# feiyue126/find_circ2

Hardware: AMD Instinct MI355X
Metric: anchor-pairs/sec (backsplice calls) at 100 bp reads, 1/2/4/8 MI355X (higher is better)
Workload: dtype u32

## Files before the change

find_circ2_amd/_native.py:

```python
from __future__ import annotations

import ctypes
import os
import subprocess

from ._lazy import LazyModule
from ._libpath import LIB_PATH, _HERE

np = LazyModule("numpy", globals(), "np")

FC2_OK = 0
CALLER_MAX_QUEUED = 64
FC2_E_PARAM = -1
FC2_E_HIP = -2
FC2_E_FORMAT = -3
FC2_E_RANGE = -4
FC2_E_IO = -5
FC2_E_KEY = -6
FC2_E_OS = -7

MAX_READ_LEN = 32767

PAIR_BACKSPLICE = 0x01
PAIR_PRIMARY_REV = 0x02
PAIR_READ_N = 0x04
PAIR_BYTEPATH = 0x08
PAIR_SKIP = 0x10
PAIR_WIN_N = 0x20
PAIR_READ_N1 = 0x40

RES_MINUS = 0x0001
RES_GTAG_SHIFT = 1
RES_GTAG_MASK = 0x1FFE
RES_ERR_KEY = 0x2000
RES_ERR_WIN = 0x4000
RES_DONE = 0x8000

_DTYPE_NAMES = ("PAIR_DTYPE", "RESULT_DTYPE", "ESCAPE_DTYPE", "LONG_PAIR_DTYPE", "LONG_RESULT_DTYPE")


def _dtypes():
    PAIR_DTYPE = np.dtype([("a_pos", "<i4"), ("b_aend", "<i4"), ("chrom", "<u4"), ("read_len", "<u2"),
                           ("flags", "u1"), ("npos", "u1")])
    RESULT_DTYPE = np.dtype([("best_x", "<i2"), ("dist", "u1"), ("ov", "u1"), ("n_ties", "<u2"), ("info", "<u2")])
    assert PAIR_DTYPE.itemsize == 16 and RESULT_DTYPE.itemsize == 8
    ESCAPE_DTYPE = np.dtype([("index", "<u8"), ("result", RESULT_DTYPE)])
    LONG_PAIR_DTYPE = np.dtype([("read_off", "<u8"), ("read_len", "<u4"), ("chrom", "<u4"), ("a_pos", "<i4"),
                                ("b_aend", "<i4"), ("flags", "u1"), ("_pad", "u1", (7,))])
    LONG_RESULT_DTYPE = np.dtype([("best_x", "<i4"), ("n_ties", "<u4"), ("dist", "u1"), ("ov", "u1"), ("info", "<u2"),
                                  ("_pad", "<u4")])
    assert LONG_PAIR_DTYPE.itemsize == 32 and LONG_RESULT_DTYPE.itemsize == 16
    g = globals()
    for k in _DTYPE_NAMES:
        g[k] = locals()[k]


def __getattr__(name):
    if name in _DTYPE_NAMES:
        _dtypes()
        return globals()[name]
    raise AttributeError("module %r has no attribute %r" % (__name__, name))
R32_ESCAPE = 0x80000000
R16_ESCAPE = 0x007F


class Fc2Error(RuntimeError):
    def __init__(self, code: int, msg: str):
        super().__init__("libfc2 error %d: %s" % (code, msg))
        self.code = code


class Params(ctypes.Structure):
    _fields_ = [("asize", ctypes.c_int32), ("margin", ctypes.c_int32), ("maxdist", ctypes.c_int32),
                ("noncanonical", ctypes.c_uint8), ("strandpref", ctypes.c_uint8),
                ("allhits", ctypes.c_uint8), ("_pad", ctypes.c_uint8)]


class GenomeView(ctypes.Structure):
    _fields_ = [("units", ctypes.c_void_p), ("nplane", ctypes.c_void_p), ("ncoarse", ctypes.c_void_p),
                ("chrom_start", ctypes.c_void_p), ("chrom_size", ctypes.c_void_p),
                ("n_units", ctypes.c_uint64), ("n_chrom", ctypes.c_uint32), ("dummy", ctypes.c_uint32),
                ("units_twin", ctypes.c_void_p), ("nsuper", ctypes.c_void_p), ("nsuper_shift", ctypes.c_uint32),
                ("nsuper_words", ctypes.c_uint32), ("wt", ctypes.c_void_p), ("wt_bytes", ctypes.c_uint64),
                ("wt_twin_off", ctypes.c_uint64)]


class BatchView(ctypes.Structure):
    _fields_ = [("pairs", ctypes.c_void_p), ("read_words", ctypes.c_void_p), ("read_nwords", ctypes.c_void_p),
                ("n", ctypes.c_uint64), ("stride", ctypes.c_uint64), ("rw", ctypes.c_uint32),
                ("nw", ctypes.c_uint32), ("max_l", ctypes.c_int32), ("layout", ctypes.c_uint32),
                ("win_words", ctypes.c_void_p), ("win_nwords", ctypes.c_void_p), ("ww", ctypes.c_uint32),
                ("wnw", ctypes.c_uint32)]


BATCH_LOCUS_ORDERED = 0x1
BATCH_FORM_STAGED = 0x02
BATCH_FORM_PLAIN = 0x04
BATCH_FORM_UNITS = 0x08
BATCH_FORM_TWOLANE = 0x10
BATCH_FORM_TRI = 0x20
BATCH_FORM_FIVE = 0x40
BATCH_FORM_WAVE = 0x80


class CompactOut(ctypes.Structure):
    _fields_ = [("width", ctypes.c_int32), ("esc_cap", ctypes.c_uint32), ("words", ctypes.c_void_p),
                ("esc", ctypes.c_void_p), ("esc_count", ctypes.c_void_p), ("count_out", ctypes.c_void_p)]


class ReorderInfo(ctypes.Structure):
    _fields_ = [("n", ctypes.c_uint64), ("workspace_bytes", ctypes.c_uint64), ("shift", ctypes.c_uint32),
                ("n_buckets", ctypes.c_uint32), ("bucket_bits", ctypes.c_uint32), ("n_chunks", ctypes.c_uint32),
                ("n_groups", ctypes.c_uint32), ("chunk", ctypes.c_uint32)]


class BytesView(ctypes.Structure):
    _fields_ = [("index", ctypes.c_void_p), ("pairs", ctypes.c_void_p), ("arena", ctypes.c_void_p),
                ("off", ctypes.c_void_p), ("m", ctypes.c_uint64)]


class SynthCfg(ctypes.Structure):
    _fields_ = [("seed", ctypes.c_uint64), ("len_min", ctypes.c_int32), ("len_max", ctypes.c_int32),
                ("p_planted", ctypes.c_float), ("p_minus_site", ctypes.c_float),
                ("p_backsplice", ctypes.c_float), ("mut_rate", ctypes.c_float), ("n_rate", ctypes.c_float),
                ("p_clip", ctypes.c_float), ("span_min", ctypes.c_int32), ("span_max", ctypes.c_int32),
                ("locus_ordered", ctypes.c_int32), ("p_three_seg", ctypes.c_float), ("first", ctypes.c_uint64)]


EXPORTED = [
    "fc2_abi_version", "fc2_last_error", "fc2_device_count", "fc2_host_register", "fc2_host_unregister", "fc2_set_tuning", "fc2_get_tuning", "fc2_max_fast_l",
    "fc2_batch_geometry",
    "fc2_bp_scan_launch", "fc2_bp_scan_bytes_launch", "fc2_probe_pattern_launch",
    "fc2_result_compact_launch", "fc2_result_expand", "fc2_bp_scan_compact_launch", "fc2_host_device_pointer",
    "fc2_fasta_open", "fc2_fasta_close", "fc2_fasta_n_chrom", "fc2_fasta_chrom", "fc2_fasta_find",
    "fc2_fasta_get_upper", "fc2_fasta_layout", "fc2_fasta_pack", "fc2_fasta_prepack",
    "fc2_pack_pairs", "fc2_bytepath_size", "fc2_bytepath_fill", "fc2_window_geometry", "fc2_pack_windows",
    "fc2_gather_windows_launch", "fc2_long_geometry", "fc2_long_fill", "fc2_bp_scan_long_launch",
    "fc2_synth_genome_launch", "fc2_coarse_launch", "fc2_twin_launch", "fc2_wtab_geometry", "fc2_wtab_launch",
    "fc2_nsuper_geometry", "fc2_nsuper_launch", "fc2_synth_pairs_launch",
    "fc2_reorder_plan", "fc2_reorder_launch",
    "fc2_ingest_open", "fc2_ingest_close", "fc2_ingest_n_refs", "fc2_ingest_ref_name", "fc2_ingest_header",
    "fc2_ingest_next", "fc2_ingest_counts_get", "fc2_ingest_set_bam_out", "fc2_ingest_close_bam_out",
    "fc2_ingest_format", "fc2_sam_to_bam", "fc2_bgzf_inflate_launch",
    "fc2_ingest_set_gpu_inflate", "fc2_ingest_set_gpu_inflate_from", "fc2_ingest_inflate_counts",
    "fc2_bam_walk_launch", "fc2_bam_walk_host", "fc2_ingest_set_gpu_walk", "fc2_ingest_walk_counts",
    "fc2_bam_digest_launch", "fc2_bam_digest_host", "fc2_ingest_set_gpu_digest", "fc2_ingest_digest_counts",
    "fc2_caller_open", "fc2_caller_set_genome", "fc2_caller_inflate_counts", "fc2_caller_ingest", "fc2_caller_close", "fc2_caller_next",
    "fc2_caller_submit", "fc2_caller_submit_compact", "fc2_caller_submit_long", "fc2_caller_queued", "fc2_caller_take", "fc2_caller_rows", "fc2_caller_write_rows", "fc2_caller_counter", "fc2_caller_stats",
    "fc2_caller_set_reads_gz", "fc2_caller_close_reads", "fc2_caller_set_reads_gz_device", "fc2_caller_reads_gz_counts",
    "fc2_deflate_launch", "fc2_deflate_scratch_bytes", "fc2_gpu_gzip", "fc2_gpu_gzip_bound", "fc2_caller_set_reads_gz_device_tuning",
    "fc2_ctx_create", "fc2_ctx_create_sibling", "fc2_ctx_destroy", "fc2_ctx_genome_load", "fc2_ctx_genome_view", "fc2_ctx_scan_async",
    "fc2_ctx_sync", "fc2_ctx_scan_long", "fc2_ctx_stream", "fc2_ctx_last_error",
]


BAM_WALK_CAP = 1824
BAM_WALK_NO_EXIT = 0xFFFFFFFF
BAM_DIGEST_MAX_BLOCKS = 1024


class BamDigest(ctypes.Structure):
    _fields_ = [("state", ctypes.c_uint8), ("as_type", ctypes.c_uint8), ("xs_type", ctypes.c_uint8),
                ("has_qual", ctypes.c_uint8), ("block_size", ctypes.c_uint32), ("astart", ctypes.c_int32),
                ("qlen", ctypes.c_int32), ("as_bits", ctypes.c_uint32), ("xs_bits", ctypes.c_uint32),
                ("aend", ctypes.c_int64)]


class IngestParams(ctypes.Structure):
    _fields_ = [("asize", ctypes.c_int32), ("nolinear", ctypes.c_uint8), ("noop", ctypes.c_uint8),
                ("_pad", ctypes.c_uint8 * 2)]


class IngestCounts(ctypes.Structure):
    _fields_ = [("n_reads", ctypes.c_uint64), ("total_mates", ctypes.c_uint64), ("unmapped_reads", ctypes.c_uint64),
                ("unspliced_mates", ctypes.c_uint64), ("seg_too_short_skip", ctypes.c_uint64),
                ("records", ctypes.c_uint64), ("handed_back", ctypes.c_uint64)]

class CallerOpts(ctypes.Structure):
    _fields_ = [("name", ctypes.c_char_p), ("known_circ", ctypes.c_char_p), ("known_lin", ctypes.c_char_p),
                ("min_uniq_qual", ctypes.c_int32), ("asize", ctypes.c_int32), ("margin", ctypes.c_int32),
                ("maxdist", ctypes.c_int32), ("short_threshold", ctypes.c_int32), ("huge_threshold", ctypes.c_int32),
                ("noncanonical", ctypes.c_uint8), ("allhits", ctypes.c_uint8), ("stranded", ctypes.c_uint8),
                ("strandpref", ctypes.c_uint8), ("halfunique", ctypes.c_uint8), ("report_nobridges", ctypes.c_uint8),
                ("test", ctypes.c_uint8), ("nolinear", ctypes.c_uint8), ("multi_events", ctypes.c_uint8),
                ("noop", ctypes.c_uint8), ("write_reads", ctypes.c_uint8), ("write_multi", ctypes.c_uint8),
                ("_pad", ctypes.c_uint32), ("chunksize", ctypes.c_uint64)]


class CallerBatch(ctypes.Structure):
    _fields_ = [("n", ctypes.c_uint64), ("reads", ctypes.c_void_p), ("read_off", ctypes.c_void_p),
                ("pairs", ctypes.c_void_p), ("n_long", ctypes.c_uint64), ("long_pairs", ctypes.c_void_p)]


_lib = None


def build(force: bool = False) -> str:
    srcdir = os.path.join(_HERE, "csrc")
    srcs = [os.path.join(srcdir, f) for f in ("fc2_kernels.hip", "fc2_scan32.hip", "fc2_reorder.hip", "fc2_inflate.hip",
                                              "fc2_deflate.hip", "fc2_deflate_gpu.hip", "fc2_deflate_gpu.h", "fc2_devcrc.h",
                                              "fc2_gzpieces.h", "fc2_scan32.h",
                                              "fc2_host.cpp", "fc2_ingest.cpp", "fc2_ingest_impl.h", "fc2_caller.cpp",
                                              "fc2_bamout.cpp", "fc2_bamout.h", "fc2_ctx.cpp", "fc2_hostmem.h",
                                              "fc2_common.h", "Makefile")]
    srcs += [os.path.join(os.path.dirname(_HERE), "include", h)
             for h in ("fc2_bp.h", "fc2_ingest.h", "fc2_caller.h", "fc2_ctx.h")]
    newest = max(os.path.getmtime(s) for s in srcs)
    if force or not os.path.exists(LIB_PATH) or os.path.getmtime(LIB_PATH) < newest:
        subprocess.check_call(["make", "-s", "-C", srcdir])
    return LIB_PATH


def lib() -> ctypes.CDLL:
    global _lib
    if _lib is not None:
        return _lib
    if not os.path.exists(LIB_PATH):
        raise ImportError("libfc2.so is not built (%s); run __graft_entry__.build() -- there is no CPU fallback"
                          % LIB_PATH)
    L = ctypes.CDLL(LIB_PATH)
    vp, u64, u32, i32, i64 = ctypes.c_void_p, ctypes.c_uint64, ctypes.c_uint32, ctypes.c_int32, ctypes.c_int64
    P = ctypes.POINTER
    sig = {
        "fc2_abi_version": (ctypes.c_int, []),
        "fc2_last_error": (ctypes.c_char_p, []),
        "fc2_device_count": (ctypes.c_int, [P(ctypes.c_int)]),
        "fc2_max_fast_l": (ctypes.c_int, []),
        "fc2_host_register": (ctypes.c_int, [vp, u64]),
        "fc2_host_unregister": (ctypes.c_int, [vp]),
        "fc2_set_tuning": (ctypes.c_int, [ctypes.c_int, ctypes.c_int]),
        "fc2_get_tuning": (ctypes.c_int, [ctypes.c_int, ctypes.POINTER(ctypes.c_int)]),
        "fc2_batch_geometry": (ctypes.c_int, [P(Params), i32, P(u32), P(u32), P(u32)]),
        "fc2_bp_scan_launch": (ctypes.c_int, [P(Params), P(GenomeView), P(BatchView), vp, vp, u32, vp]),
        "fc2_bp_scan_bytes_launch": (ctypes.c_int, [P(Params), P(BytesView), vp, vp, u32, u64, vp]),
        "fc2_probe_pattern_launch": (ctypes.c_int, [P(Params), P(GenomeView), P(BatchView), vp, vp]),
        "fc2_result_compact_launch": (ctypes.c_int, [P(Params), vp, u64, ctypes.c_int, vp, vp, u32, vp, vp]),
        "fc2_result_expand": (ctypes.c_int, [P(Params), vp, ctypes.c_int, u64, vp, u64, vp, ctypes.c_int]),
        "fc2_bp_scan_compact_launch": (ctypes.c_int, [P(Params), P(GenomeView), P(BatchView), P(CompactOut), vp]),
        "fc2_host_device_pointer": (ctypes.c_int, [vp, P(vp)]),
        "fc2_fasta_open": (ctypes.c_int, [ctypes.c_char_p, ctypes.c_int, P(vp)]),
        "fc2_fasta_close": (None, [vp]),
        "fc2_fasta_n_chrom": (ctypes.c_int, [vp]),
        "fc2_fasta_chrom": (ctypes.c_int, [vp, ctypes.c_int, P(ctypes.c_char_p), P(i64), P(i64), P(i64),
                                           P(i64), P(ctypes.c_int)]),
        "fc2_fasta_find": (ctypes.c_int, [vp, ctypes.c_char_p]),
        "fc2_fasta_get_upper": (ctypes.c_int, [vp, ctypes.c_int, i64, i64, vp, i64, P(i64)]),
        "fc2_fasta_layout": (ctypes.c_int, [vp, P(u64), P(u64), vp]),
        "fc2_fasta_pack": (ctypes.c_int, [vp, vp, vp, vp, P(u64), ctypes.c_int]),
        "fc2_fasta_prepack": (ctypes.c_int, [vp, ctypes.c_int]),
        "fc2_pack_pairs": (ctypes.c_int, [P(Params), vp, u64, vp, vp, vp, vp, u32, vp, u32, u64, P(u64),
                                          ctypes.c_int]),
        "fc2_bytepath_size": (ctypes.c_int, [P(Params), u64, vp, P(u64), P(u64)]),
        "fc2_window_geometry": (ctypes.c_int, [P(Params), ctypes.c_int, P(u32), P(u32), P(u32)]),
        "fc2_pack_windows": (ctypes.c_int, [P(Params), vp, u64, vp, vp, vp, u32, u64, ctypes.c_int]),
        "fc2_gather_windows_launch": (ctypes.c_int, [P(Params), P(GenomeView), P(BatchView), vp, vp, vp, u32, vp]),
        "fc2_bytepath_fill": (ctypes.c_int, [P(Params), vp, u64, vp, vp, vp, vp, vp, vp, vp]),
        "fc2_long_geometry": (ctypes.c_int, [P(Params), u64, vp, P(ctypes.c_uint64), vp]),
        "fc2_long_fill": (ctypes.c_int, [P(Params), vp, u64, vp, vp, vp, vp]),
        "fc2_bp_scan_long_launch": (ctypes.c_int, [P(Params), u64, vp, vp, vp, vp, vp, vp, vp]),
        "fc2_synth_genome_launch": (ctypes.c_int, [u64, vp, vp, vp, u64, vp, vp, u32, vp]),
        "fc2_coarse_launch": (ctypes.c_int, [vp, vp, u64, vp]),
        "fc2_twin_launch": (ctypes.c_int, [vp, u64, vp, vp]),
        "fc2_wtab_geometry": (ctypes.c_int, [u64, P(u64), P(u64)]),
        "fc2_wtab_launch": (ctypes.c_int, [vp, u64, vp, vp]),
        "fc2_nsuper_geometry": (ctypes.c_int, [u64, P(u32), P(u32)]),
        "fc2_nsuper_launch": (ctypes.c_int, [vp, u64, vp, vp]),
        "fc2_synth_pairs_launch": (ctypes.c_int, [P(Params), P(SynthCfg), P(GenomeView), vp, u64, vp, vp, u32,
                                                  vp, u32, u64, vp, vp]),
        "fc2_reorder_plan": (ctypes.c_int, [P(GenomeView), u64, P(ReorderInfo)]),
        "fc2_reorder_launch": (ctypes.c_int, [P(ReorderInfo), P(GenomeView), P(BatchView), vp, vp, vp, vp, vp, vp]),
        "fc2_ingest_open": (ctypes.c_int, [ctypes.c_char_p, ctypes.c_int, P(vp)]),
        "fc2_ingest_close": (None, [vp]),
        "fc2_ingest_n_refs": (ctypes.c_int, [vp]),
        "fc2_ingest_ref_name": (ctypes.c_char_p, [vp, ctypes.c_int]),
        "fc2_ingest_header": (ctypes.c_char_p, [vp]),
        "fc2_ingest_next": (ctypes.c_int, [vp, P(IngestParams), u64, P(IngestCounts), P(ctypes.c_void_p), P(u64),
                                           P(u64), P(ctypes.c_int)]),
        "fc2_ingest_counts_get": (ctypes.c_int, [vp, P(IngestCounts)]),
        "fc2_ingest_set_bam_out": (ctypes.c_int, [vp, ctypes.c_char_p]),
        "fc2_ingest_close_bam_out": (ctypes.c_int, [vp]),
        "fc2_ingest_format": (ctypes.c_int, [vp, P(ctypes.c_int)]),
        "fc2_sam_to_bam": (ctypes.c_int, [ctypes.c_char_p, ctypes.c_char_p]),
        "fc2_caller_open": (ctypes.c_int, [ctypes.c_char_p, ctypes.c_int, P(CallerOpts), P(vp)]),
        "fc2_caller_set_genome": (ctypes.c_int, [vp, vp, i32, vp, P(u64), P(u64)]),
        "fc2_caller_ingest": (vp, [vp]),
        "fc2_caller_close": (None, [vp]),
        "fc2_caller_next": (ctypes.c_int, [vp, P(CallerBatch), P(ctypes.c_int)]),
        "fc2_caller_submit": (ctypes.c_int, [vp, vp, vp, u32, u64]),
        "fc2_caller_submit_compact": (ctypes.c_int, [vp, vp, ctypes.c_int, u64, vp, u64, vp, u32, u64]),
        "fc2_caller_submit_long": (ctypes.c_int, [vp, vp, u64, vp, u64]),
        "fc2_caller_queued": (ctypes.c_int, [vp]),
        "fc2_caller_take": (ctypes.c_int, [vp, ctypes.c_int, P(ctypes.c_void_p), P(u64)]),
        "fc2_caller_set_reads_gz": (ctypes.c_int, [vp, ctypes.c_char_p, ctypes.c_int, ctypes.c_int, u64]),
        "fc2_caller_close_reads": (ctypes.c_int, [vp]),
        "fc2_caller_set_reads_gz_device": (ctypes.c_int, [vp, ctypes.c_int]),
        "fc2_caller_reads_gz_counts": (ctypes.c_int, [vp, P(u64), P(u64)]),
        "fc2_deflate_launch": (ctypes.c_int, [vp, u64, u32, vp, u32, vp, vp, vp, vp]),
        "fc2_deflate_scratch_bytes": (u64, [u64, u32]),
        "fc2_gpu_gzip": (ctypes.c_int, [ctypes.c_int, vp, u64, u32, vp, u64, P(u64)]),
        "fc2_gpu_gzip_bound": (u64, [u64, u32]),
        "fc2_caller_set_reads_gz_device_tuning": (ctypes.c_int, [vp, u32, ctypes.c_double]),
        "fc2_caller_rows": (ctypes.c_int, [vp, ctypes.c_int, P(ctypes.c_void_p), P(u64)]),
        "fc2_caller_write_rows": (ctypes.c_int, [vp, ctypes.c_int, ctypes.c_int, P(u64)]),
        "fc2_caller_counter": (ctypes.c_int, [vp, ctypes.c_int, P(ctypes.c_char_p), P(ctypes.c_double)]),
        "fc2_caller_stats": (ctypes.c_int, [vp, P(u64), P(u64)]),
        "fc2_bgzf_inflate_launch": (ctypes.c_int, [vp, vp, vp, vp, vp, vp, vp, u32, vp]),
        "fc2_ingest_set_gpu_inflate": (ctypes.c_int, [vp, ctypes.c_int, ctypes.c_int]),
        "fc2_ingest_set_gpu_inflate_from": (ctypes.c_int, [vp, ctypes.c_int, u64]),
        "fc2_ingest_inflate_counts": (ctypes.c_int, [vp, P(u64), P(u64)]),
        "fc2_bam_walk_launch": (ctypes.c_int, [vp, vp, vp, vp, vp, vp, u32, vp]),
        "fc2_bam_walk_host": (ctypes.c_int, [vp, u32, vp, P(u32), P(u32)]),
        "fc2_ingest_set_gpu_walk": (ctypes.c_int, [vp, ctypes.c_int]),
        "fc2_ingest_walk_counts": (ctypes.c_int, [vp, P(u64), P(u64)]),
        "fc2_bam_digest_launch": (ctypes.c_int, [vp, u32, vp, vp, vp, vp, vp, vp, vp, u32, vp]),
        "fc2_bam_digest_host": (ctypes.c_int, [vp, u32, u32, P(BamDigest)]),
        "fc2_ingest_set_gpu_digest": (ctypes.c_int, [vp, ctypes.c_int]),
        "fc2_ingest_digest_counts": (ctypes.c_int, [vp, P(u64), P(u64)]),
        "fc2_caller_inflate_counts": (ctypes.c_int, [vp, P(u64), P(u64)]),
        "fc2_ctx_create": (ctypes.c_int, [ctypes.c_int, P(vp)]),
        "fc2_ctx_create_sibling": (ctypes.c_int, [vp, P(vp)]),
        "fc2_ctx_destroy": (None, [vp]),
        "fc2_ctx_genome_load": (ctypes.c_int, [vp, vp, ctypes.c_int]),
        "fc2_ctx_genome_view": (ctypes.c_int, [vp, P(GenomeView)]),
        "fc2_ctx_scan_async": (ctypes.c_int, [vp, P(Params), u64, vp, vp, vp, vp, vp, u32, ctypes.c_int]),
        "fc2_ctx_sync": (ctypes.c_int, [vp]),
        "fc2_ctx_scan_long": (ctypes.c_int, [vp, P(Params), u64, vp, vp, vp, vp]),
        "fc2_ctx_stream": (vp, [vp]),
        "fc2_ctx_last_error": (ctypes.c_char_p, [vp]),
    }
    for name, (res, args) in sig.items():
        if os.environ.get("FC2_LIB_VARIANT") and not hasattr(L, name):
            continue
        fn = getattr(L, name)
        fn.restype = res
        fn.argtypes = args
    if L.fc2_abi_version() != 1:
        raise ImportError("libfc2.so ABI mismatch")
    _lib = L
    return L


def get_tuning(key: int) -> int:
    v = ctypes.c_int(0)
    check(lib().fc2_get_tuning(key, ctypes.byref(v)))
    return v.value


def check(rc: int) -> None:
    if rc != FC2_OK:
        msg = lib().fc2_last_error()
        raise Fc2Error(rc, msg.decode("utf-8", "replace") if msg else "")


def ptr(a) -> int:
    if a is None:
        return None
    if isinstance(a, np.ndarray):
        return a.ctypes.data
    return a.data_ptr()
```

find_circ2_amd/csrc/fc2_ctx.cpp:

```cpp
#include <hip/hip_runtime.h>
#include <stdio.h>
#include <stdlib.h>
#include <string.h>
#include <sys/mman.h>

#include <algorithm>
#include <chrono>
#include <memory>
#include <string>
#include <vector>

#include "../../include/fc2_bp.h"
#include "../../include/fc2_ctx.h"
#include "fc2_common.h"
#include "fc2_hostmem.h"

namespace {

int hip_fail(hipError_t e, const char *what) {
    return fc2::fail(FC2_E_HIP, std::string(what) + ": " + hipGetErrorString(e));
}

struct DevBuf {
    void *p = nullptr;
    size_t cap = 0;
    int reserve(size_t bytes, const char *what, bool slack = true) {
        if (bytes <= cap && p) return FC2_OK;
        if (p) (void)hipFree(p);
        p = nullptr;
        cap = 0;
        const size_t want = std::max<size_t>(slack ? bytes + bytes / 4 : bytes, 256);
        const hipError_t e = hipMalloc(&p, want);
        if (e != hipSuccess) { p = nullptr; return hip_fail(e, what); }
        cap = want;
        return FC2_OK;
    }
    void release() {
        if (p) (void)hipFree(p);
        p = nullptr;
        cap = 0;
    }
    template <class T> T *as() const { return static_cast<T *>(p); }
};

struct HostBuf {
    void *p = nullptr;
    size_t cap = 0;
    int reserve(size_t bytes, const char *what) {
        if (bytes <= cap && p) return FC2_OK;
        if (p) (void)hipHostFree(p);
        p = nullptr;
        cap = 0;
        const size_t want = std::max<size_t>(bytes + bytes / 4, 256);
        const hipError_t e = hipHostMalloc(&p, want, hipHostMallocDefault);
        if (e != hipSuccess) { p = nullptr; return hip_fail(e, what); }
        cap = want;
        return FC2_OK;
    }
    void release() {
        if (p) (void)hipHostFree(p);
        p = nullptr;
        cap = 0;
    }
    template <class T> T *as() const { return static_cast<T *>(p); }
};

}

struct fc2_ctx {
    int device = 0;
    hipStream_t stream = nullptr;
    std::string err;
    bool have_genome = false;
    bool borrowed = false;
    const fc2_fasta *fa = nullptr;
    fc2_genome_view gv{};
    DevBuf units, nplane, ncoarse, cstart, csize, twin, nsuper, wt;
    fc2::MappedWords h_units, h_nplane;
    HostBuf h_pairs, h_words, h_nwords, h_res, h_tm, h_bidx, h_bpairs, h_boff, h_arena;
    DevBuf d_pairs, d_words, d_nwords, d_res, d_tm, d_bidx, d_bpairs, d_boff, d_arena;
    bool pending = false;
    uint64_t n = 0;
    uint32_t tw = 0;
    bool allhits = false;
    fc2_result *out_res = nullptr;
    uint64_t *out_tm = nullptr;

    void free_genome() {
        if (!borrowed)
            for (DevBuf *b : {&units, &nplane, &ncoarse, &cstart, &csize, &twin, &nsuper, &wt}) b->release();
        h_units.release();
        h_nplane.release();
        borrowed = false;
        gv = fc2_genome_view{};
        have_genome = false;
        fa = nullptr;
    }
};

namespace {

int keep(fc2_ctx *c, int rc) {
    if (rc != FC2_OK && c) {
        const char *m = fc2_last_error();
        c->err = m ? m : "";
    }
    return rc;
}

int use_device(fc2_ctx *c) {
    const hipError_t e = hipSetDevice(c->device);
    return e == hipSuccess ? FC2_OK : hip_fail(e, "hipSetDevice");
}

int h2d(DevBuf &d, const void *src, size_t bytes, hipStream_t s) {
    if (!bytes) return FC2_OK;
    const hipError_t e = hipMemcpyAsync(d.p, src, bytes, hipMemcpyHostToDevice, s);
    return e == hipSuccess ? FC2_OK : hip_fail(e, "hipMemcpyAsync H2D");
}

}

extern "C" int fc2_ctx_create(int device, fc2_ctx **out) {
    if (!out) return fc2::fail(FC2_E_PARAM, "fc2_ctx_create: null argument");
    *out = nullptr;
    if (device < 0) return fc2::fail(FC2_E_PARAM, "fc2_ctx_create: negative device");
    int count = 0;
    hipError_t e = hipGetDeviceCount(&count);
    if (e != hipSuccess) return hip_fail(e, "fc2_ctx_create: hipGetDeviceCount");
    if (device >= count)
        return fc2::fail(FC2_E_HIP, "fc2_ctx_create: device " + std::to_string(device) + " of " +
                                        std::to_string(count));
    fc2_ctx *c = new fc2_ctx();
    c->device = device;
    int rc = use_device(c);
    if (rc == FC2_OK) {
        e = hipStreamCreateWithFlags(&c->stream, hipStreamNonBlocking);
        if (e != hipSuccess) rc = hip_fail(e, "hipStreamCreateWithFlags");
    }
    if (rc != FC2_OK) {
        delete c;
        return rc;
    }
    *out = c;
    return FC2_OK;
}

extern "C" int fc2_ctx_create_sibling(const fc2_ctx *src, fc2_ctx **out) {
    if (!src || !out) return fc2::fail(FC2_E_PARAM, "fc2_ctx_create_sibling: null argument");
    *out = nullptr;
    if (!src->have_genome) return fc2::fail(FC2_E_PARAM, "fc2_ctx_create_sibling: the source context has no genome");
    fc2_ctx *c = nullptr;
    if (int rc = fc2_ctx_create(src->device, &c)) return rc;
    c->gv = src->gv;
    c->fa = src->fa;
    c->have_genome = true;
    c->borrowed = true;
    *out = c;
    return FC2_OK;
}

extern "C" void fc2_ctx_destroy(fc2_ctx *c) {
    if (!c) return;
    if (hipSetDevice(c->device) == hipSuccess && c->stream) (void)hipStreamSynchronize(c->stream);
    c->free_genome();
    for (HostBuf *b : {&c->h_pairs, &c->h_words, &c->h_nwords, &c->h_res, &c->h_tm, &c->h_bidx, &c->h_bpairs,
                       &c->h_boff, &c->h_arena})
        b->release();
    for (DevBuf *b : {&c->d_pairs, &c->d_words, &c->d_nwords, &c->d_res, &c->d_tm, &c->d_bidx, &c->d_bpairs,
                      &c->d_boff, &c->d_arena})
        b->release();
    if (c->stream) (void)hipStreamDestroy(c->stream);
    delete c;
}

extern "C" int fc2_ctx_genome_load(fc2_ctx *c, const fc2_fasta *fa, int n_threads) {
    if (!c) return fc2::fail(FC2_E_PARAM, "fc2_ctx_genome_load: null context");
    c->err.clear();
    if (c->pending) return keep(c, fc2::fail(FC2_E_PARAM, "fc2_ctx_genome_load: a batch is queued (fc2_ctx_sync)"));
    int rc = use_device(c);
    if (rc) return keep(c, rc);
    if (hipStreamSynchronize(c->stream) != hipSuccess) return keep(c, fc2::fail(FC2_E_HIP, "stream sync"));
    c->free_genome();
    if (!fa) {
        c->gv.dummy = 1;
        c->gv.n_chrom = 0xFFFFFFFFu;
        c->have_genome = true;
        return FC2_OK;
    }
    static const bool timing = getenv("FC2_CALLER_TIMING") != nullptr;
    const auto t0 = std::chrono::steady_clock::now();
    auto ms = [&] { return std::chrono::duration<double, std::milli>(std::chrono::steady_clock::now() - t0).count(); };
    const int nch = fc2_fasta_n_chrom(fa);
    std::vector<int64_t> sizes((size_t)std::max(nch, 1), 0);
    for (int i = 0; i < nch; ++i)
        if ((rc = fc2_fasta_chrom(fa, i, nullptr, &sizes[(size_t)i], nullptr, nullptr, nullptr, nullptr))) return keep(c, rc);
    uint64_t nu = 0, ncw = 0;
    std::vector<uint64_t> cs((size_t)std::max(nch, 1), 0);
    if ((rc = fc2_fasta_layout(fa, &nu, &ncw, cs.data()))) return keep(c, rc);
    fc2::MappedWords &units = c->h_units, &nplane = c->h_nplane;
    std::vector<uint32_t> ncoarse;
    uint64_t n_exotic = 0;
    const bool prepacked = fc2::take_prepacked(fa, nu, units, nplane, ncoarse);
    if (!prepacked) {
        units = fc2::MappedWords(2 * nu);
        nplane = fc2::MappedWords(nu);
    }
    if (!units.ok() || !nplane.ok()) return keep(c, fc2::fail(FC2_E_OS, "fc2_ctx_genome_load: cannot map host memory for the 2-bit genome"));
    const double t_alloc = ms();
    if (!prepacked) {
        ncoarse.assign((size_t)std::max<uint64_t>(ncw, 1), 0);
        if ((rc = fc2_fasta_pack(fa, units.data(), nplane.data(), ncoarse.data(), &n_exotic, n_threads))) return keep(c, rc);
    }
    const double t_pack = ms();
    const hipStream_t s = c->stream;
    if ((rc = c->units.reserve(units.size() * 8, "genome units", false)) || (rc = c->nplane.reserve(nplane.size() * 8, "genome N plane", false)) ||
        (rc = c->ncoarse.reserve(ncoarse.size() * 4, "genome coarse N map", false)) || (rc = c->cstart.reserve(cs.size() * 8, "chromosome starts", false)) ||
        (rc = c->csize.reserve(sizes.size() * 8, "chromosome sizes", false)) || (rc = c->twin.reserve(2 * (nu + 8) * 8, "genome twin", false)))
        return keep(c, rc);
    if ((rc = h2d(c->units, units.data(), units.size() * 8, s)) || (rc = h2d(c->nplane, nplane.data(), nplane.size() * 8, s)) ||
        (rc = h2d(c->ncoarse, ncoarse.data(), ncoarse.size() * 4, s)) || (rc = h2d(c->cstart, cs.data(), cs.size() * 8, s)) ||
        (rc = h2d(c->csize, sizes.data(), sizes.size() * 8, s)))
        return keep(c, rc);
    if ((rc = fc2_twin_launch(c->units.as<uint64_t>(), nu, c->twin.as<uint64_t>(), s))) return keep(c, rc);
    uint32_t ns_shift = 0, ns_words = 0;
    if ((rc = fc2_nsuper_geometry(nu, &ns_shift, &ns_words))) return keep(c, rc);
    const size_t ns_alloc = ((size_t)ns_words + 3) / 4 * 4;
    if ((rc = c->nsuper.reserve(ns_alloc * 4, "N super map", false))) return keep(c, rc);
    if (hipMemsetAsync(c->nsuper.p, 0, ns_alloc * 4, s) != hipSuccess) return keep(c, fc2::fail(FC2_E_HIP, "memset"));
    if ((rc = fc2_nsuper_launch(c->ncoarse.as<uint32_t>(), nu, c->nsuper.as<uint32_t>(), s))) return keep(c, rc);
    uint64_t wt_bytes = 0, wt_twin_off = 0;
    const bool words = fc2_wtab_geometry(nu, &wt_bytes, &wt_twin_off) == FC2_OK;
    if (words) {
        if ((rc = c->wt.reserve(wt_bytes, "word-pair table", false))) return keep(c, rc);
        if ((rc = fc2_wtab_launch(c->units.as<uint64_t>(), nu, c->wt.as<uint32_t>(), s))) return keep(c, rc);
    }
    const hipError_t e = hipStreamSynchronize(s);
    if (e != hipSuccess) return keep(c, hip_fail(e, "genome upload"));
    if (timing)
        fprintf(stderr, "genome load: host vectors %.1f ms, 2-bit pack %.1f ms%s, device alloc + upload + tables %.1f ms "
                        "(%llu units)\n", t_alloc, t_pack - t_alloc, prepacked ? " (prepacked)" : "", ms() - t_pack,
                (unsigned long long)nu);
    fc2_genome_view &g = c->gv;
    g.units = c->units.as<const uint64_t>();
    g.nplane = c->nplane.as<const uint64_t>();
    g.ncoarse = c->ncoarse.as<const uint32_t>();
    g.chrom_start = c->cstart.as<const uint64_t>();
    g.chrom_size = c->csize.as<const int64_t>();
    g.n_units = nu;
    g.n_chrom = (uint32_t)nch;
    g.dummy = 0;
    g.units_twin = c->twin.as<const uint64_t>();
    g.nsuper = c->nsuper.as<const uint32_t>();
    g.nsuper_shift = ns_shift;
    g.nsuper_words = ns_words;
    g.wt = words ? c->wt.as<const uint32_t>() : nullptr;
    g.wt_bytes = words ? wt_bytes : 0;
    g.wt_twin_off = words ? wt_twin_off : 0;
    c->fa = fa;
    c->have_genome = true;
    return FC2_OK;
}

extern "C" int fc2_ctx_genome_view(const fc2_ctx *c, fc2_genome_view *out) {
    if (!c || !out) return fc2::fail(FC2_E_PARAM, "fc2_ctx_genome_view: null argument");
    if (!c->have_genome) return fc2::fail(FC2_E_PARAM, "fc2_ctx_genome_view: no genome loaded");
    *out = c->gv;
    return FC2_OK;
}

extern "C" int fc2_ctx_scan_async(fc2_ctx *c, const fc2_params *p, uint64_t n, const uint8_t *reads,
                                  const uint64_t *read_off, const fc2_pair *pairs, fc2_result *results,
                                  uint64_t *tiemask, uint32_t tw, int n_threads) {
    if (!c) return fc2::fail(FC2_E_PARAM, "fc2_ctx_scan_async: null context");
    c->err.clear();
    int rc = fc2::validate_params(p);
    if (rc) return keep(c, rc);
    if (c->pending) return keep(c, fc2::fail(FC2_E_PARAM, "fc2_ctx_scan_async: the previous batch was not synced"));
    if (!c->have_genome)
        return keep(c, fc2::fail(FC2_E_PARAM, "fc2_ctx_scan_async: no genome (fc2_ctx_genome_load; NULL = dummy genome)"));
    if (n && (!reads || !read_off || !pairs || !results))
        return keep(c, fc2::fail(FC2_E_PARAM, "fc2_ctx_scan_async: null argument"));
    if (p->allhits && n && !tiemask) return keep(c, fc2::fail(FC2_E_PARAM, "fc2_ctx_scan_async: --all-hits needs a tie mask"));
    if ((rc = use_device(c))) return keep(c, rc);
    c->n = n;
    c->allhits = p->allhits != 0;
    c->tw = tw;
    c->out_res = results;
    c->out_tm = tiemask;
    if (n == 0) {
        c->pending = true;
        return FC2_OK;
    }
    int max_len = 0;
    for (uint64_t i = 0; i < n; ++i) max_len = std::max<int>(max_len, pairs[i].read_len);
    uint32_t rw = 0, nw = 0, tw_need = 0;
    if ((rc = fc2_batch_geometry(p, max_len, &rw, &nw, &tw_need))) return keep(c, rc);
    if (c->allhits && tw < tw_need)
        return keep(c, fc2::fail(FC2_E_PARAM, "fc2_ctx_scan_async: tie mask of " + std::to_string(tw) + " words per pair, " +
                                                  std::to_string(tw_need) + " needed"));
    const size_t tmw = c->allhits ? (size_t)tw * n : 0;
    if ((rc = c->h_pairs.reserve(n * sizeof(fc2_pair), "pair staging")) || (rc = c->h_words.reserve((size_t)rw * n * 8, "read-row staging")) ||
        (rc = c->h_nwords.reserve((size_t)nw * n * 8, "N-row staging")) || (rc = c->h_res.reserve(n * 8, "result staging")) ||
        (tmw && (rc = c->h_tm.reserve(tmw * 8, "tie-mask staging"))) || (rc = c->d_pairs.reserve(n * sizeof(fc2_pair), "pairs")) ||
        (rc = c->d_words.reserve((size_t)rw * n * 8, "read rows")) || (rc = c->d_nwords.reserve((size_t)nw * n * 8, "N rows")) ||
        (rc = c->d_res.reserve(n * 8, "results")) || (tmw && (rc = c->d_tm.reserve(tmw * 8, "tie mask"))))
        return keep(c, rc);
    memcpy(c->h_pairs.p, pairs, n * sizeof(fc2_pair));
    memset(c->h_words.p, 0, (size_t)rw * n * 8);
    memset(c->h_nwords.p, 0, (size_t)nw * n * 8);
    fc2_pair *hp = c->h_pairs.as<fc2_pair>();
    uint64_t n_bytepath = 0;
    if ((rc = fc2_pack_pairs(p, c->fa, n, reads, read_off, hp, c->h_words.as<uint64_t>(), rw, c->h_nwords.as<uint64_t>(), nw,
                             n, &n_bytepath, n_threads)))
        return keep(c, rc);
    const int e = fc2::eff_anchor(p);
    int max_l = 0;
    for (uint64_t i = 0; i < n; ++i)
        if (!(hp[i].flags & (FC2_PAIR_BYTEPATH | FC2_PAIR_SKIP))) max_l = std::max(max_l, (int)hp[i].read_len - 2 * e);
    const hipStream_t s = c->stream;
    auto abandon = [&](int code) {
        const std::string msg = fc2_last_error();
        (void)hipStreamSynchronize(s);
        return keep(c, fc2::fail(code, msg));
    };
    if ((rc = h2d(c->d_pairs, hp, n * sizeof(fc2_pair), s)) || (rc = h2d(c->d_words, c->h_words.p, (size_t)rw * n * 8, s)) ||
        (rc = h2d(c->d_nwords, c->h_nwords.p, (size_t)nw * n * 8, s)))
        return abandon(rc);
    if (tmw && hipMemsetAsync(c->d_tm.p, 0, tmw * 8, s) != hipSuccess) return abandon(fc2::fail(FC2_E_HIP, "tie-mask memset"));
    fc2_batch_view bv{};
    bv.pairs = c->d_pairs.as<const fc2_pair>();
    bv.read_words = c->d_words.as<const uint64_t>();
    bv.read_nwords = c->d_nwords.as<const uint64_t>();
    bv.n = n;
    bv.stride = n;
    bv.rw = rw;
    bv.nw = nw;
    bv.max_l = max_l;
    bv.layout = 0;
    uint64_t *dtm = tmw ? c->d_tm.as<uint64_t>() : nullptr;
    if ((rc = fc2_bp_scan_launch(p, &c->gv, &bv, c->d_res.as<fc2_result>(), dtm, tw, s))) return abandon(rc);
    if (n_bytepath) {
        uint64_t m = 0, arena = 0;
        if ((rc = fc2_bytepath_size(p, n, hp, &m, &arena))) return abandon(rc);
        if ((rc = c->h_bidx.reserve(m * 8, "byte-path index")) || (rc = c->h_bpairs.reserve(m * sizeof(fc2_pair), "byte-path pairs")) ||
            (rc = c->h_boff.reserve(m * 8, "byte-path offsets")) || (rc = c->h_arena.reserve(std::max<uint64_t>(arena, 16), "byte-path arena")) ||
            (rc = c->d_bidx.reserve(m * 8, "byte-path index")) || (rc = c->d_bpairs.reserve(m * sizeof(fc2_pair), "byte-path pairs")) ||
            (rc = c->d_boff.reserve(m * 8, "byte-path offsets")) || (rc = c->d_arena.reserve(std::max<uint64_t>(arena, 16), "byte-path arena")))
            return abandon(rc);
        if ((rc = fc2_bytepath_fill(p, c->fa, n, reads, read_off, hp, c->h_bidx.as<uint64_t>(), c->h_bpairs.as<fc2_pair>(),
                                    c->h_boff.as<uint64_t>(), c->h_arena.as<uint8_t>())))
            return abandon(rc);
        if ((rc = h2d(c->d_bidx, c->h_bidx.p, m * 8, s)) || (rc = h2d(c->d_bpairs, c->h_bpairs.p, m * sizeof(fc2_pair), s)) ||
            (rc = h2d(c->d_boff, c->h_boff.p, m * 8, s)) || (rc = h2d(c->d_arena, c->h_arena.p, arena, s)))
            return abandon(rc);
        fc2_bytes_view v{c->d_bidx.as<const uint64_t>(), c->d_bpairs.as<const fc2_pair>(), c->d_arena.as<const uint8_t>(),
                         c->d_boff.as<const uint64_t>(), m};
        if ((rc = fc2_bp_scan_bytes_launch(p, &v, c->d_res.as<fc2_result>(), dtm, tw, n, s))) return abandon(rc);
    }
    hipError_t he = hipMemcpyAsync(c->h_res.p, c->d_res.p, n * 8, hipMemcpyDeviceToHost, s);
    if (he == hipSuccess && tmw) he = hipMemcpyAsync(c->h_tm.p, c->d_tm.p, tmw * 8, hipMemcpyDeviceToHost, s);
    if (he != hipSuccess) return abandon(hip_fail(he, "hipMemcpyAsync D2H"));
    c->pending = true;
    return FC2_OK;
}

extern "C" int fc2_ctx_sync(fc2_ctx *c) {
    if (!c) return fc2::fail(FC2_E_PARAM, "fc2_ctx_sync: null context");
    c->err.clear();
    if (!c->pending) return FC2_OK;
    c->pending = false;
    int rc = use_device(c);
    if (rc) return keep(c, rc);
    const hipError_t e = hipStreamSynchronize(c->stream);
    if (e != hipSuccess) return keep(c, hip_fail(e, "fc2_ctx_sync"));
    if (c->n) {
        memcpy(c->out_res, c->h_res.p, c->n * 8);
        if (c->allhits) memcpy(c->out_tm, c->h_tm.p, (size_t)c->tw * c->n * 8);
    }
    return FC2_OK;
}

extern "C" int fc2_ctx_scan_long(fc2_ctx *c, const fc2_params *p, uint64_t n, const uint8_t *reads,
                                 const fc2_long_pair *pairs, fc2_long_result *results, uint64_t *ties) {
    if (!c) return fc2::fail(FC2_E_PARAM, "fc2_ctx_scan_long: null context");
    c->err.clear();
    int rc = fc2::validate_params(p);
    if (rc) return keep(c, rc);
    if (c->pending) return keep(c, fc2::fail(FC2_E_PARAM, "fc2_ctx_scan_long: a batch is queued (fc2_ctx_sync)"));
    if (!c->have_genome)
        return keep(c, fc2::fail(FC2_E_PARAM, "fc2_ctx_scan_long: no genome (fc2_ctx_genome_load; NULL = dummy genome)"));
    if (n == 0) return FC2_OK;
    if (!reads || !pairs || !results || (p->allhits && !ties))
        return keep(c, fc2::fail(FC2_E_PARAM, "fc2_ctx_scan_long: null argument"));
    if ((rc = use_device(c))) return keep(c, rc);
    uint64_t arena = 0;
    std::vector<uint64_t> tie_off(n + 1), off(n);
    if ((rc = fc2_long_geometry(p, n, pairs, &arena, tie_off.data()))) return keep(c, rc);
    std::vector<uint8_t> h_arena((size_t)std::max<uint64_t>(arena, 16));
    if ((rc = fc2_long_fill(p, c->fa, n, reads, pairs, off.data(), h_arena.data()))) return keep(c, rc);
    const uint64_t nt = p->allhits ? tie_off[n] : 0;
    DevBuf d_lp, d_off, d_arena, d_toff, d_res, d_ties;
    auto cleanup = [&] { for (DevBuf *b : {&d_lp, &d_off, &d_arena, &d_toff, &d_res, &d_ties}) b->release(); };
    const hipStream_t s = c->stream;
    if ((rc = d_lp.reserve(n * sizeof(fc2_long_pair), "long pairs", false)) || (rc = d_off.reserve(n * 8, "long offsets", false)) ||
        (rc = d_arena.reserve(h_arena.size(), "long arena", false)) || (rc = d_toff.reserve((n + 1) * 8, "long tie offsets", false)) ||
        (rc = d_res.reserve(n * sizeof(fc2_long_result), "long results", false)) ||
        (nt && (rc = d_ties.reserve(nt * 8, "long ties", false)))) {
        cleanup();
        return keep(c, rc);
    }
    if ((rc = h2d(d_lp, pairs, n * sizeof(fc2_long_pair), s)) || (rc = h2d(d_off, off.data(), n * 8, s)) ||
        (rc = h2d(d_arena, h_arena.data(), h_arena.size(), s)) || (rc = h2d(d_toff, tie_off.data(), (n + 1) * 8, s)) ||
        (rc = fc2_bp_scan_long_launch(p, n, d_lp.as<fc2_long_pair>(), d_off.as<uint64_t>(), d_arena.as<uint8_t>(),
                                      d_toff.as<uint64_t>(), d_res.as<fc2_long_result>(), nt ? d_ties.as<uint64_t>() : nullptr, s))) {
        (void)hipStreamSynchronize(s);
        cleanup();
        return keep(c, rc);
    }
    hipError_t he = hipMemcpyAsync(results, d_res.p, n * sizeof(fc2_long_result), hipMemcpyDeviceToHost, s);
    if (he == hipSuccess && nt) he = hipMemcpyAsync(ties, d_ties.p, nt * 8, hipMemcpyDeviceToHost, s);
    const hipError_t se = hipStreamSynchronize(s);
    cleanup();
    if (he != hipSuccess) return keep(c, hip_fail(he, "fc2_ctx_scan_long D2H"));
    if (se != hipSuccess) return keep(c, hip_fail(se, "fc2_ctx_scan_long"));
    return FC2_OK;
}

extern "C" void *fc2_ctx_stream(const fc2_ctx *c) { return c ? (void *)c->stream : nullptr; }

extern "C" const char *fc2_ctx_last_error(const fc2_ctx *c) { return c ? c->err.c_str() : ""; }
```

find_circ2_amd/csrc/fc2_host.cpp:

```cpp
#include <errno.h>
#include <fcntl.h>
#include <stdio.h>
#include <stdlib.h>
#include <string.h>
#include <sys/mman.h>
#include <sys/stat.h>
#include <unistd.h>
#include <immintrin.h>

#include <algorithm>
#include <atomic>
#include <chrono>
#include <functional>
#include <memory>
#include <string>
#include <thread>
#include <unordered_map>
#include <vector>

#include "fc2_common.h"
#include "fc2_compact.h"
#include "fc2_hostmem.h"

namespace fc2 {

static thread_local std::string g_err;

void set_error(const std::string &msg) { g_err = msg; }
int fail(int code, const std::string &msg) {
    g_err = msg;
    return code;
}

int validate_params(const fc2_params *p) {
    if (!p) return fail(FC2_E_PARAM, "null fc2_params");
    if ((int64_t)p->asize - p->margin < -65536)
        return fail(FC2_E_RANGE, "asize - margin < -65536 is not supported (windows of over 128k bases per pair)");
    if (p->margin > 255) return fail(FC2_E_RANGE, "margin > 255 is not supported (ov is stored in 8 bits)");
    return FC2_OK;
}

static int n_workers(int n_threads) {
    if (n_threads > 0) return n_threads;
    unsigned h = std::thread::hardware_concurrency();
    const char *env = getenv("OMP_NUM_THREADS");
    if (env && atoi(env) > 0) h = (unsigned)atoi(env);
    if (h == 0) h = 1;
    if (h > 64) h = 64;
    return (int)h;
}

static void parallel_for(uint64_t n, int threads, const std::function<void(uint64_t, uint64_t)> &body) {
    if (n == 0) return;
    if (threads <= 1 || n < 4096) {
        body(0, n);
        return;
    }
    uint64_t t = (uint64_t)threads;
    if (t > n) t = n;
    std::vector<std::thread> pool;
    pool.reserve(t);
    for (uint64_t k = 0; k < t; ++k) {
        const uint64_t b = n * k / t, e = n * (k + 1) / t;
        pool.emplace_back([&body, b, e] { body(b, e); });
    }
    for (auto &th : pool) th.join();
}

static inline uint8_t upc(uint8_t c) { return (c >= 'a' && c <= 'z') ? (uint8_t)(c - 32) : c; }

static inline int bclass(uint8_t c) {
    switch (upc(c)) {
        case 'A': return 0;
        case 'C': return 1;
        case 'G': return 2;
        case 'T': return 3;
        case 'N': return 4;
        default: return 5;
    }
}

struct PackTable {
    uint8_t t[256];
    PackTable() {
        for (int c = 0; c < 256; ++c) {
            const int cl = bclass((uint8_t)c);
            t[c] = (uint8_t)(cl < 4 ? cl : cl == 4 ? 4 : 4 | 8);
        }
    }
};
static const PackTable kPackTable;
static inline uint32_t pack_code(uint8_t c) { return kPackTable.t[c]; }

struct BaseMasks {
    uint64_t a, c, g, t, n, nl;
};

static inline BaseMasks base_masks_scalar(const uint8_t *s, int len) {
    BaseMasks m{0, 0, 0, 0, 0, 0};
    for (int j = 0; j < len; ++j) {
        const uint64_t bit = 1ull << j;
        if (s[j] == '\n') m.nl |= bit;
        switch (s[j] & 0xDF) {
            case 'A': m.a |= bit; break;
            case 'C': m.c |= bit; break;
            case 'G': m.g |= bit; break;
            case 'T': m.t |= bit; break;
            case 'N': m.n |= bit; break;
            default: break;
        }
    }
    return m;
}

__attribute__((target("avx2"))) static BaseMasks base_masks_avx2(const uint8_t *s) {
    const __m256i up = _mm256_set1_epi8((char)0xDF);
    const __m256i r0 = _mm256_loadu_si256((const __m256i *)s), r1 = _mm256_loadu_si256((const __m256i *)(s + 32));
    const __m256i v0 = _mm256_and_si256(r0, up), v1 = _mm256_and_si256(r1, up);
#define FC2_MASK64(x0, x1, ch)                                                                             \
    ((uint64_t)(uint32_t)_mm256_movemask_epi8(_mm256_cmpeq_epi8(x0, _mm256_set1_epi8(ch))) |                 \
     (uint64_t)(uint32_t)_mm256_movemask_epi8(_mm256_cmpeq_epi8(x1, _mm256_set1_epi8(ch))) << 32)
    const BaseMasks m{FC2_MASK64(v0, v1, 'A'), FC2_MASK64(v0, v1, 'C'), FC2_MASK64(v0, v1, 'G'),
                      FC2_MASK64(v0, v1, 'T'), FC2_MASK64(v0, v1, 'N'), FC2_MASK64(r0, r1, '\n')};
#undef FC2_MASK64
    return m;
}

#if defined(__HIP_DEVICE_COMPILE__)
static const bool kHaveAvx2 = false;
#else
static const bool kHaveAvx2 = (__builtin_cpu_init(), __builtin_cpu_supports("avx2"));
#endif

static inline bool acgt8(uint64_t u) {
    auto zero = [](uint64_t y) { return ~(((y & 0x7F7F7F7F7F7F7F7Full) + 0x7F7F7F7F7F7F7F7Full) | y | 0x7F7F7F7F7F7F7F7Full); };
    const uint64_t m = zero(u ^ 0x4141414141414141ull) | zero(u ^ 0x4343434343434343ull) |
                       zero(u ^ 0x4747474747474747ull) | zero(u ^ 0x5454545454545454ull);
    return m == 0x8080808080808080ull;
}

static inline bool py_isspace(uint8_t c) {
    return c == ' ' || c == '\t' || c == '\n' || c == '\r' || c == '\v' || c == '\f';
}

}

using namespace fc2;

struct fc2_chrom_rec {
    std::string name;
    int64_t ofs = 0, ldata = 0, skip = 0, size = 0;
    std::string skipchar;
    int nfields = 4;
    int regular = -1;
    uint64_t gstart = 0;
};

struct fc2_fasta {
    std::string path;
    int fd = -1;
    const uint8_t *data = nullptr;
    size_t n = 0;
    std::vector<fc2_chrom_rec> chroms;
    std::unordered_map<std::string, int> by_name;
    std::vector<uint64_t> exotic;
    bool packed = false;
    struct Prepacked {
        fc2::MappedWords units, nplane;
        std::vector<uint32_t> ncoarse;
        uint64_t n_units = 0;
    };
    std::unique_ptr<Prepacked> prepacked;
};

static int build_index(fc2_fasta *f) {
    std::unordered_map<std::string, int> &idx = f->by_name;
    std::vector<fc2_chrom_rec> &cs = f->chroms;
    int64_t ofs = 0, chrom_ofs = 0, size = 0;
    std::string chrom = "undef";
    const uint8_t *d = f->data;
    const size_t n = f->n;
    size_t i = 0;
    while (i < n) {
        const uint8_t *nl = (const uint8_t *)memchr(d + i, '\n', n - i);
        const size_t j = nl ? (size_t)(nl - d) + 1 : n;
        const uint8_t *line = d + i;
        const int64_t len = (int64_t)(j - i);
        ofs += len;
        if (line[0] == '>') {
            if (size) {
                auto it = idx.find(chrom);
                if (it == idx.end())
                    return fail(FC2_E_FORMAT, "FASTA header without sequence before '" + chrom +
                                                  "': reference indexed_fasta.index raises KeyError");
                cs[it->second].size = size;
                cs[it->second].nfields += 1;
            }
            int64_t s = 1;
            while (s < len && py_isspace(line[s])) ++s;
            int64_t e = s;
            while (e < len && !py_isspace(line[e])) ++e;
            if (e == s) return fail(FC2_E_FORMAT, "empty FASTA header: reference raises IndexError");
            chrom.assign((const char *)line + s, (size_t)(e - s));
            chrom_ofs = ofs;
        } else {
            int64_t a = 0, b = len;
            while (a < b && py_isspace(line[a])) ++a;
            while (b > a && py_isspace(line[b - 1])) --b;
            const int64_t stripped = b - a;
            if (idx.find(chrom) == idx.end()) {
                size = 0;
                fc2_chrom_rec r;
                r.name = chrom;
                r.ofs = chrom_ofs;
                r.ldata = stripped;
                r.skip = len - stripped;
                r.skipchar.assign((const char *)line + stripped, (size_t)(len - stripped));
                idx[chrom] = (int)cs.size();
                cs.push_back(r);
            }
            size += stripped;
        }
        i = j;
    }
    if (size) {
        auto it = idx.find(chrom);
        if (it != idx.end()) {
            cs[it->second].size = size;
            cs[it->second].nfields += 1;
        }
    }
    for (auto &c : cs)
        if (c.nfields != 5)
            return fail(FC2_E_FORMAT, "chromosome '" + c.name +
                                          "' has an inconsistent index entry (empty or duplicated sequence); "
                                          "the reference's store_index/get_data fail on it");
    return FC2_OK;
}

static std::string py2_repr(const std::string &s) {
    std::string o = "'";
    for (unsigned char c : s) {
        if (c == '\n') o += "\\n";
        else if (c == '\r') o += "\\r";
        else if (c == '\t') o += "\\t";
        else if (c == '\'') o += "\\'";
        else if (c == '\\') o += "\\\\";
        else if (c >= 32 && c < 127) o += (char)c;
        else {
            char buf[8];
            snprintf(buf, sizeof buf, "\\x%02x", c);
            o += buf;
        }
    }
    return o + "'";
}

static bool py2_unescape(const std::string &in, std::string &out) {
    out.clear();
    for (size_t i = 0; i < in.size(); ++i) {
        char c = in[i];
        if (c != '\\') { out += c; continue; }
        if (++i >= in.size()) return false;
        switch (in[i]) {
            case 'n': out += '\n'; break;
            case 'r': out += '\r'; break;
            case 't': out += '\t'; break;
            case '\\': out += '\\'; break;
            case '\'': out += '\''; break;
            case '"': out += '"'; break;
            case 'x': {
                if (i + 2 >= in.size()) return false;
                out += (char)strtol(in.substr(i + 1, 2).c_str(), nullptr, 16);
                i += 2;
                break;
            }
            default: out += '\\'; out += in[i];
        }
    }
    return true;
}

static int load_index_file(fc2_fasta *f, const std::string &ipath) {
    FILE *fp = fopen(ipath.c_str(), "r");
    if (!fp) return fail(FC2_E_IO, "cannot open index: IOError: [Errno " + std::to_string(errno) + "] " +
                                       strerror(errno) + ": '" + ipath + "'");
    char *line = nullptr;
    size_t cap = 0;
    ssize_t len;
    int rc = FC2_OK;
    while ((len = getline(&line, &cap, fp)) > 0) {
        std::string s(line, (size_t)len);
        while (!s.empty() && py_isspace((uint8_t)s.back())) s.pop_back();
        std::vector<std::string> parts;
        size_t st = 0;
        for (;;) {
            size_t t = s.find('\t', st);
            parts.push_back(s.substr(st, t == std::string::npos ? std::string::npos : t - st));
            if (t == std::string::npos) break;
            st = t + 1;
        }
        if (parts.size() != 6 || parts[4].size() < 2) { rc = fail(FC2_E_FORMAT, "malformed .byo_index line: " + s); break; }
        fc2_chrom_rec r;
        r.name = parts[0];
        r.ofs = atoll(parts[1].c_str());
        r.ldata = atoll(parts[2].c_str());
        r.skip = atoll(parts[3].c_str());
        if (!py2_unescape(parts[4].substr(1, parts[4].size() - 2), r.skipchar)) { rc = fail(FC2_E_FORMAT, "bad skipchar in .byo_index"); break; }
        r.size = atoll(parts[5].c_str());
        r.nfields = 5;
        f->by_name[r.name] = (int)f->chroms.size();
        f->chroms.push_back(r);
    }
    free(line);
    fclose(fp);
    std::stable_sort(f->chroms.begin(), f->chroms.end(),
                     [](const fc2_chrom_rec &a, const fc2_chrom_rec &b) { return a.ofs < b.ofs; });
    f->by_name.clear();
    for (size_t i = 0; i < f->chroms.size(); ++i) f->by_name[f->chroms[i].name] = (int)i;
    return rc;
}

static int store_index_file(const fc2_fasta *f, const std::string &ipath) {
    std::vector<const fc2_chrom_rec *> v;
    for (auto &c : f->chroms) v.push_back(&c);
    std::sort(v.begin(), v.end(), [](const fc2_chrom_rec *a, const fc2_chrom_rec *b) { return a->name < b->name; });
    std::string dir = ipath.substr(0, ipath.find_last_of('/') == std::string::npos ? 0 : ipath.find_last_of('/') + 1);
    std::string tmpl = (dir.empty() ? std::string("./") : dir) + "tmpXXXXXX";
    std::vector<char> buf(tmpl.begin(), tmpl.end());
    buf.push_back(0);
    auto oserror = [&](int err, const char *what) {
        return fail(FC2_E_OS, std::string("OSError: [Errno ") + std::to_string(err) + "] " + strerror(err) + ": '" +
                                  what + "' (writing the FASTA index " + ipath + ")");
    };
    int fd = mkstemp(buf.data());
    if (fd < 0) return oserror(errno, tmpl.c_str());
    std::string body;
    for (auto *c : v) {
        char num[128];
        body += c->name;
        snprintf(num, sizeof num, "\t%lld\t%lld\t%lld\t", (long long)c->ofs, (long long)c->ldata, (long long)c->skip);
        body += num;
        body += py2_repr(c->skipchar);
        snprintf(num, sizeof num, "\t%lld\n", (long long)c->size);
        body += num;
    }
    size_t done = 0;
    while (done < body.size()) {
        const ssize_t w = write(fd, body.data() + done, body.size() - done);
        if (w < 0) {
            if (errno == EINTR) continue;
            const int err = errno;
            close(fd);
            unlink(buf.data());
            return oserror(err, buf.data());
        }
        done += (size_t)w;
    }
    if (fsync(fd) != 0) { const int err = errno; close(fd); unlink(buf.data()); return oserror(err, buf.data()); }
    close(fd);
    if (chmod(buf.data(), S_IRUSR | S_IRGRP | S_IROTH) != 0) { const int err = errno; unlink(buf.data()); return oserror(err, buf.data()); }
    if (rename(buf.data(), ipath.c_str()) != 0) { const int err = errno; unlink(buf.data()); return oserror(err, buf.data()); }
    return FC2_OK;
}

static inline int64_t floordiv(int64_t a, int64_t b) {
    int64_t q = a / b;
    if ((a % b != 0) && ((a < 0) != (b < 0))) --q;
    return q;
}
static inline int64_t pyclip(int64_t i, int64_t n) {
    if (i < 0) { i += n; if (i < 0) i = 0; }
    return i > n ? n : i;
}

static int get_upper_impl(const fc2_fasta *f, int ci, int64_t start, int64_t end, std::string &out,
                          size_t limit = SIZE_MAX, int64_t *full_len = nullptr, int tail_char = -1,
                          int64_t *tail_mis = nullptr) {
    out.clear();
    if (tail_mis) *tail_mis = 0;
    if (!f) {
        if (end > start) out.assign(std::min((size_t)(end - start), limit), 'N');
        const int64_t full = end > start ? end - start : 0;
        if (full_len) *full_len = full;
        if (tail_mis && tail_char != 'N' && full > (int64_t)limit) *tail_mis = full - (int64_t)limit;
        return FC2_OK;
    }
    if (ci < 0 || ci >= (int)f->chroms.size()) return fail(FC2_E_KEY, "unknown chromosome index");
    const fc2_chrom_rec &c = f->chroms[ci];
    if (c.ldata == 0) return fail(FC2_E_FORMAT, "chromosome '" + c.name + "' has ldata 0: reference raises ZeroDivisionError");
    int64_t pad_start = 0, pad_end = 0;
    if (start < 0) { pad_start = -start; start = 0; }
    if (end > c.size) { pad_end = end - c.size; end = c.size; }
    const int64_t os = pyclip(floordiv(start, c.ldata) * c.skip + start + c.ofs, (int64_t)f->n);
    const int64_t oe = pyclip(floordiv(end, c.ldata) * c.skip + end + c.ofs, (int64_t)f->n);
    const uint64_t full = (uint64_t)pad_start + (uint64_t)pad_end + (uint64_t)(oe > os ? oe - os : 0);
    if (limit == SIZE_MAX && full > (1ull << 32))
        return fail(FC2_E_RANGE, "window of " + std::to_string(full) + " bytes from chromosome '" + c.name +
                                     "': the reference's get_data raises MemoryError");
    out.reserve(std::min((size_t)full, limit));
    out.append(std::min((size_t)pad_start, limit), 'N');
    const size_t sl = c.skipchar.size();
    for (int64_t p = os; p < oe && out.size() < limit;) {
        if (sl && p + (int64_t)sl <= oe && !memcmp(f->data + p, c.skipchar.data(), sl)) { p += (int64_t)sl; continue; }
        out.push_back((char)upc(f->data[p]));
        ++p;
    }
    out.append(std::min((size_t)pad_end, limit - out.size()), 'N');
    if (full_len || tail_mis) {
        const int64_t lim = limit == SIZE_MAX ? INT64_MAX : (int64_t)limit;
        int64_t k = pad_start, mis = 0;
        const bool n_differs = tail_char != 'N';
        if (n_differs && pad_start > lim) mis += pad_start - lim;
        for (int64_t p = os; p < oe;) {
            if (sl && p + (int64_t)sl <= oe && !memcmp(f->data + p, c.skipchar.data(), sl)) { p += (int64_t)sl; continue; }
            if (k >= lim && (int)upc(f->data[p]) != tail_char) ++mis;
            ++k;
            ++p;
        }
        if (n_differs) mis += std::max<int64_t>(0, k + pad_end - std::max(k, lim));
        if (full_len) *full_len = k + pad_end;
        if (tail_mis) *tail_mis = mis;
    }
    return FC2_OK;
}

extern "C" int fc2_abi_version(void) { return FC2_ABI_VERSION; }
extern "C" const char *fc2_last_error(void) { return g_err.c_str(); }
extern "C" int fc2_max_fast_l(void) { return kMaxFastL; }

extern "C" int fc2_batch_geometry(const fc2_params *p, int32_t max_read_len, uint32_t *rw, uint32_t *nw, uint32_t *tw) {
    int rc = validate_params(p);
    if (rc) return rc;
    int lmax = max_read_len - 2 * eff_anchor(p);
    if (lmax < 0) lmax = 0;
    const int lfast = lmax > kMaxFastL ? kMaxFastL : lmax;
    if (rw) *rw = (uint32_t)std::max(1, (2 * lfast + 63) / 64);
    if (nw) *nw = (uint32_t)std::max(1, (lfast + 63) / 64);
    if (tw) *tw = (uint32_t)(2 * std::max(1, (lmax + 2 + 63) / 64));
    return FC2_OK;
}

extern "C" int fc2_fasta_open(const char *path, int write_index, fc2_fasta **out) {
    if (!path || !out) return fail(FC2_E_PARAM, "fc2_fasta_open: null argument");
    *out = nullptr;
    auto ioerror = [&](int err) {
        return fail(FC2_E_IO, std::string("cannot open FASTA: IOError: [Errno ") + std::to_string(err) + "] " +
                                  strerror(err) + ": '" + path + "'");
    };
    int fd = open(path, O_RDONLY);
    if (fd < 0) return ioerror(errno);
    struct stat st;
    if (fstat(fd, &st) != 0) { const int err = errno; close(fd); return ioerror(err); }
    if (S_ISDIR(st.st_mode)) { close(fd); return ioerror(EISDIR); }
    fc2_fasta *f = new fc2_fasta();
    f->path = path;
    f->fd = fd;
    f->n = (size_t)st.st_size;
    if (f->n) {
        void *m = mmap(nullptr, f->n, PROT_READ, MAP_SHARED, fd, 0);
        if (m == MAP_FAILED) {
            const int err = errno;
            close(fd);
            delete f;
            return fail(FC2_E_OS, std::string("mmap.error: [Errno ") + std::to_string(err) + "] " + strerror(err) +
                                      " (FASTA '" + path + "')");
        }
        f->data = (const uint8_t *)m;
        madvise(m, f->n, MADV_WILLNEED);
    }
    const std::string ipath = std::string(path) + ".byo_index";
    int rc;
    if (access(ipath.c_str(), R_OK) == 0) {
        rc = load_index_file(f, ipath);
    } else {
        rc = build_index(f);
        if (rc == FC2_OK && write_index) rc = store_index_file(f, ipath);
    }
    if (rc != FC2_OK) { fc2_fasta_close(f); return rc; }
    *out = f;
    return FC2_OK;
}

extern "C" void fc2_fasta_close(fc2_fasta *f) {
    if (!f) return;
    if (f->data) munmap((void *)f->data, f->n);
    if (f->fd >= 0) close(f->fd);
    delete f;
}

extern "C" int fc2_fasta_n_chrom(const fc2_fasta *f) { return f ? (int)f->chroms.size() : 0; }

extern "C" int fc2_fasta_chrom(const fc2_fasta *f, int i, const char **name, int64_t *size, int64_t *ofs, int64_t *ldata,
                               int64_t *skip, int *regular) {
    if (!f || i < 0 || i >= (int)f->chroms.size()) return fail(FC2_E_PARAM, "fc2_fasta_chrom: bad index");
    const fc2_chrom_rec &c = f->chroms[i];
    if (name) *name = c.name.c_str();
    if (size) *size = c.size;
    if (ofs) *ofs = c.ofs;
    if (ldata) *ldata = c.ldata;
    if (skip) *skip = c.skip;
    if (regular) *regular = c.regular;
    return FC2_OK;
}

extern "C" int fc2_fasta_find(const fc2_fasta *f, const char *name) {
    if (!f || !name) return -1;
    auto it = f->by_name.find(name);
    return it == f->by_name.end() ? -1 : it->second;
}

extern "C" int fc2_fasta_get_upper(const fc2_fasta *f, int chrom, int64_t start, int64_t end, uint8_t *out, int64_t cap,
                                   int64_t *len) {
    std::string s;
    int rc = get_upper_impl(f, chrom, start, end, s);
    if (rc) return rc;
    if (len) *len = (int64_t)s.size();
    if (out && cap > 0) memcpy(out, s.data(), (size_t)std::min<int64_t>(cap, (int64_t)s.size()));
    return FC2_OK;
}

static bool compute_layout(fc2_fasta *f, uint64_t *n_units) {
    constexpr uint64_t kMaxBases = 1ull << 40;
    uint64_t g = 0;
    for (auto &c : f->chroms) {
        c.gstart = g;
        const uint64_t sz = (uint64_t)std::max<int64_t>(c.size, 0);
        if (sz > kMaxBases || g + sz > kMaxBases) return false;
        g += (sz + 63) & ~63ull;
    }
    *n_units = std::max<uint64_t>(1, g / 64);
    return true;
}

extern "C" int fc2_fasta_layout(const fc2_fasta *cf, uint64_t *n_units, uint64_t *n_coarse_words, uint64_t *chrom_start) {
    if (!cf) return fail(FC2_E_PARAM, "fc2_fasta_layout: null");
    fc2_fasta *f = const_cast<fc2_fasta *>(cf);
    uint64_t nu;
    if (!compute_layout(f, &nu))
        return fail(FC2_E_RANGE, "fc2_fasta_layout: chromosome sizes add up to more than 2^40 bases (a damaged index?)");
    if (n_units) *n_units = nu;
    if (n_coarse_words) *n_coarse_words = (((nu + 15) >> 4) + 31) >> 5;
    if (chrom_start)
        for (size_t i = 0; i < f->chroms.size(); ++i) chrom_start[i] = f->chroms[i].gstart;
    return FC2_OK;
}

static bool chrom_rows_in_file(const fc2_fasta *f, const fc2_chrom_rec &c) {
    if (c.size <= 0) return true;
    if (c.ldata <= 0) return false;
    if ((int64_t)c.skipchar.size() != c.skip) return false;
    const int64_t n = (int64_t)f->n;
    if (c.ofs < 0 || c.ofs > n || c.ldata > n || c.size > n) return false;
    for (char ch : c.skipchar)
        if (!py_isspace((uint8_t)ch)) return false;
    const int64_t nfull = c.size / c.ldata, rem = c.size % c.ldata;
    int64_t stride, last;
    if (__builtin_add_overflow(c.ldata, c.skip, &stride) ||
        __builtin_mul_overflow(rem ? nfull : nfull - 1, stride, &last) ||
        __builtin_add_overflow(last, c.ofs + (rem ? rem : c.ldata), &last))
        return false;
    return last <= n;
}

extern "C" int fc2_fasta_pack(const fc2_fasta *cf, uint64_t *units, uint64_t *nplane, uint32_t *ncoarse,
                              uint64_t *n_exotic, int n_threads) {
    if (!cf || !units || !nplane || !ncoarse) return fail(FC2_E_PARAM, "fc2_fasta_pack: null argument");
    fc2_fasta *f = const_cast<fc2_fasta *>(cf);
    uint64_t nu;
    if (!compute_layout(f, &nu))
        return fail(FC2_E_RANGE, "fc2_fasta_pack: chromosome sizes add up to more than 2^40 bases (a damaged index?)");
    const int T = n_workers(n_threads);
    static const bool timing = getenv("FC2_CALLER_TIMING") != nullptr;
    const auto t0 = std::chrono::steady_clock::now();
    auto ms = [&] { return std::chrono::duration<double, std::milli>(std::chrono::steady_clock::now() - t0).count(); };
    std::vector<uint8_t> regular(f->chroms.size());
    for (size_t c = 0; c < f->chroms.size(); ++c) regular[c] = chrom_rows_in_file(f, f->chroms[c]) ? 1 : 0;
    std::unique_ptr<std::atomic<uint8_t>[]> broken(new std::atomic<uint8_t>[std::max<size_t>(1, f->chroms.size())]);
    for (size_t c = 0; c < f->chroms.size(); ++c) broken[c].store(0, std::memory_order_relaxed);
    const double t_regular = ms();
    struct Item { int c; uint64_t u0, u1; };
    std::vector<Item> items;
    for (int c = 0; c < (int)f->chroms.size(); ++c) {
        const fc2_chrom_rec &r = f->chroms[c];
        const uint64_t cu = ((uint64_t)std::max<int64_t>(r.size, 0) + 63) / 64;
        for (uint64_t u = 0; u < cu; u += 16384) items.push_back({c, u, std::min(cu, u + 16384)});
    }
    uint64_t covered = 0;
    for (const fc2_chrom_rec &r : f->chroms) covered += ((uint64_t)std::max<int64_t>(r.size, 0) + 63) / 64;
    for (uint64_t u = covered; u < nu; ++u) { units[2 * u] = 0; units[2 * u + 1] = 0; nplane[u] = ~0ull; }
    std::vector<std::vector<uint64_t>> exo(items.size());
    std::atomic<size_t> next{0};
    std::vector<std::thread> pool;
    for (int t = 0; t < std::max(1, std::min<int>(T, (int)items.size())); ++t)
        pool.emplace_back([&] {
            for (size_t k; (k = next.fetch_add(1)) < items.size();) {
                const Item it = items[k];
                const fc2_chrom_rec &r = f->chroms[it.c];
                const uint64_t gu0 = r.gstart / 64;
                if (regular[(size_t)it.c] != 1) {
                    for (uint64_t u = it.u0; u < it.u1; ++u) {
                        units[2 * (gu0 + u)] = 0;
                        units[2 * (gu0 + u) + 1] = 0;
                        nplane[gu0 + u] = ~0ull;
                    }
                    continue;
                }
                const int64_t ld = r.ldata;
                int64_t p = (int64_t)it.u0 * 64;
                const int64_t pend = std::min<int64_t>((int64_t)it.u1 * 64, r.size);
                int64_t col = p % ld;
                const uint8_t *src = f->data + r.ofs + (p / ld) * (ld + r.skip) + col;
                const uint8_t *const fend = f->data + f->n;
                uint64_t u = gu0 + it.u0, lo = 0, hi = 0, nn = 0;
                int b = 0;
                bool bad = false;
                while (p < pend) {
                    const int seg = (int)std::min<int64_t>(std::min<int64_t>(ld - col, pend - p), 64 - b);
                    const BaseMasks m = (kHaveAvx2 && fend - src >= 64) ? base_masks_avx2(src) : base_masks_scalar(src, seg);
                    const uint64_t keep = seg == 64 ? ~0ull : (1ull << seg) - 1;
                    bad |= (m.nl & keep) != 0;
                    const uint64_t acgt = m.a | m.c | m.g | m.t;
                    lo |= ((m.c | m.t) & keep) << b;
                    hi |= ((m.g | m.t) & keep) << b;
                    nn |= (~acgt & keep) << b;
                    for (uint64_t ex = ~(acgt | m.n) & keep; ex; ex &= ex - 1)
                        exo[k].push_back(r.gstart + (uint64_t)p + (uint64_t)__builtin_ctzll(ex));
                    b += seg;
                    p += seg;
                    src += seg;
                    col += seg;
                    if (col == ld) {
                        const int64_t te = src - f->data;
                        const bool sep = te + r.skip <= (int64_t)f->n &&
                                         memcmp(src, r.skipchar.data(), (size_t)r.skip) == 0;
                        bad |= !(sep || (p == r.size && te == (int64_t)f->n));
                        col = 0;
                        src += r.skip;
                    }
                    if (b == 64 || p == pend) {
                        if (b < 64) nn |= ~0ull << b;
                        units[2 * u] = lo;
                        units[2 * u + 1] = hi;
                        nplane[u] = nn;
                        ++u;
                        lo = hi = nn = 0;
                        b = 0;
                    }
                }
                if (bad) broken[it.c].store(1, std::memory_order_relaxed);
            }
        });
    for (auto &th : pool) th.join();
    for (size_t k = 0; k < items.size(); ++k) {
        const Item it = items[k];
        if (!broken[it.c].load(std::memory_order_relaxed)) continue;
        regular[(size_t)it.c] = 0;
        const uint64_t gu0 = f->chroms[it.c].gstart / 64;
        for (uint64_t u = it.u0; u < it.u1; ++u) {
            units[2 * (gu0 + u)] = 0;
            units[2 * (gu0 + u) + 1] = 0;
            nplane[gu0 + u] = ~0ull;
        }
        exo[k].clear();
    }
    for (size_t c = 0; c < f->chroms.size(); ++c) f->chroms[c].regular = regular[c];
    const double t_planes = ms();
    f->exotic.clear();
    for (auto &v : exo) f->exotic.insert(f->exotic.end(), v.begin(), v.end());
    const uint64_t n_blocks = (nu + 15) >> 4, n_words = (n_blocks + 31) >> 5;
    parallel_for(n_words, T, [&](uint64_t b, uint64_t e) {
        for (uint64_t w = b; w < e; ++w) {
            uint32_t bits = 0;
            for (int k = 0; k < 32; ++k) {
                const uint64_t blk = w * 32 + k;
                if (blk >= n_blocks) break;
                uint64_t acc = 0;
                for (int j = 0; j < 16; ++j) {
                    const uint64_t u = blk * 16 + j;
                    if (u < nu) acc |= nplane[u];
                }
                if (acc) bits |= 1u << k;
            }
            ncoarse[w] = bits;
        }
    });
    if (n_exotic) *n_exotic = f->exotic.size();
    if (timing)
        fprintf(stderr, "fasta pack: layout check %.1f ms, planes + row check %.1f ms, coarse N map %.1f ms (%d threads)\n", t_regular,
                t_planes - t_regular, ms() - t_planes, T);
    f->packed = true;
    return FC2_OK;
}

extern "C" int fc2_fasta_prepack(fc2_fasta *f, int n_threads) {
    if (!f) return fail(FC2_E_PARAM, "fc2_fasta_prepack: null");
    uint64_t nu = 0, ncw = 0;
    if (int rc = fc2_fasta_layout(f, &nu, &ncw, nullptr)) return rc;
    std::unique_ptr<fc2_fasta::Prepacked> pp(new fc2_fasta::Prepacked);
    pp->units = fc2::MappedWords(2 * nu);
    pp->nplane = fc2::MappedWords(nu);
    if (!pp->units.ok() || !pp->nplane.ok())
        return fail(FC2_E_OS, "fc2_fasta_prepack: cannot map host memory for the 2-bit genome");
    pp->ncoarse.assign((size_t)std::max<uint64_t>(ncw, 1), 0);
    uint64_t n_exotic = 0;
    if (int rc = fc2_fasta_pack(f, pp->units.data(), pp->nplane.data(), pp->ncoarse.data(), &n_exotic, n_threads)) return rc;
    pp->n_units = nu;
    f->prepacked = std::move(pp);
    return FC2_OK;
}

bool fc2::take_prepacked(const fc2_fasta *cf, uint64_t n_units, MappedWords &units, MappedWords &nplane,
                         std::vector<uint32_t> &ncoarse) {
    fc2_fasta *f = const_cast<fc2_fasta *>(cf);
    if (!f || !f->prepacked || f->prepacked->n_units != n_units) return false;
    units = std::move(f->prepacked->units);
    nplane = std::move(f->prepacked->nplane);
    ncoarse.swap(f->prepacked->ncoarse);
    f->prepacked.reset();
    return true;
}

static bool touches_exotic(const fc2_fasta *f, uint64_t g0, uint64_t g1) {
    if (f->exotic.empty() || g1 <= g0) return false;
    auto it = std::lower_bound(f->exotic.begin(), f->exotic.end(), g0);
    return it != f->exotic.end() && *it < g1;
}

extern "C" int fc2_pack_pairs(const fc2_params *p, const fc2_fasta *f, uint64_t n, const uint8_t *reads,
                              const uint64_t *read_off, fc2_pair *pairs, uint64_t *read_words, uint32_t rw,
                              uint64_t *read_nwords, uint32_t nw, uint64_t stride, uint64_t *n_bytepath,
                              int n_threads) {
    int rc = validate_params(p);
    if (rc) return rc;
    if (n && (!reads || !read_off || !pairs || !read_words || !read_nwords)) return fail(FC2_E_PARAM, "fc2_pack_pairs: null argument");
    if (stride < n) return fail(FC2_E_PARAM, "fc2_pack_pairs: stride < n");
    if (f && !f->packed) return fail(FC2_E_PARAM, "fc2_pack_pairs: genome must be packed first (fc2_fasta_pack)");
    const int e = eff_anchor(p);
    const int T = n_workers(n_threads);
    std::atomic<uint64_t> nbp{0};
    std::atomic<int64_t> bad_chrom{-1}, bad_rows{-1}, bad_dist{-1}, bad_len{-1};
    const int nch = f ? (int)f->chroms.size() : 0;
    const int maxdist = p->maxdist;
    parallel_for(n, T, [&](uint64_t b, uint64_t en) {
        uint64_t local_bp = 0;
        constexpr int kW = (kMaxFastL + 63) / 64;
        for (uint64_t i = b; i < en; ++i) {
            fc2_pair &pr = pairs[i];
            uint8_t flags = (uint8_t)(pr.flags & (FC2_PAIR_BACKSPLICE | FC2_PAIR_PRIMARY_REV | FC2_PAIR_SKIP));
            uint8_t npos = 0;
            uint64_t row[2 * kW + 1] = {0}, nrow[kW] = {0};
            const int L = pr.read_len;
            const int l = L - 2 * e;
            bool bytepath = false;
            do {
                if (flags & FC2_PAIR_SKIP) break;
                if (L > FC2_MAX_READ_LEN) { int64_t x = -1; bad_len.compare_exchange_strong(x, (int64_t)i); break; }
                if (f && (int)pr.chrom >= nch) { int64_t x = -1; bad_chrom.compare_exchange_strong(x, (int64_t)i); break; }
                if (l < 0) break;
                if (maxdist > 255 && l > 255) { int64_t x = -1; bad_dist.compare_exchange_strong(x, (int64_t)i); }
                if (e <= 0) { bytepath = true; break; }
                if (l > kMaxFastL) { bytepath = true; break; }
                if ((uint64_t)2 * l > (uint64_t)rw * 64 || (uint64_t)l > (uint64_t)nw * 64) {
                    int64_t x = -1; bad_rows.compare_exchange_strong(x, (int64_t)i); break;
                }
                const uint8_t *I = reads + read_off[i] + e;
                uint64_t lo_w[kW] = {0}, hi_w[kW] = {0}, n_w[kW] = {0};
                uint32_t any = 0;
                int j = 0;
                for (; j + 8 <= l; j += 8) {
                    uint64_t x;
                    memcpy(&x, I + j, 8);
                    const uint64_t u = x & 0xDFDFDFDFDFDFDFDFull;
                    if (!acgt8(u)) break;
                    const uint64_t v = ((x >> 2) ^ (x >> 1)) & 0x0303030303030303ull;
                    const uint64_t lo8 = ((v & 0x0101010101010101ull) * 0x0102040810204080ull) >> 56;
                    const uint64_t hi8 = (((v >> 1) & 0x0101010101010101ull) * 0x0102040810204080ull) >> 56;
                    lo_w[j >> 6] |= lo8 << (j & 63);
                    hi_w[j >> 6] |= hi8 << (j & 63);
                }
                for (; j < l; ++j) {
                    const uint32_t pc = pack_code(I[j]);
                    const uint64_t bit = 1ull << (j & 63);
                    if (pc & 4u) n_w[j >> 6] |= bit;
                    else {
                        if (pc & 1u) lo_w[j >> 6] |= bit;
                        if (pc & 2u) hi_w[j >> 6] |= bit;
                    }
                    any |= pc;
                }
                if (any & 8u) { bytepath = true; break; }
                const int nlw = (l + 63) / 64;
                for (int k = 0; k < nlw; ++k) row[k] = lo_w[k];
                const int sh = l & 63, wo = l >> 6;
                for (int k = 0; k < nlw; ++k) {
                    row[wo + k] |= sh ? (hi_w[k] << sh) : hi_w[k];
                    if (sh) row[wo + k + 1] |= hi_w[k] >> (64 - sh);
                }
                if (any & 4u) {
                    int n_count = 0, n_first = 0;
                    for (int k = 0; k < nlw; ++k) {
                        nrow[k] = n_w[k];
                        if (n_w[k]) {
                            if (n_count == 0) n_first = k * 64 + __builtin_ctzll(n_w[k]);
                            n_count += __builtin_popcountll(n_w[k]);
                        }
                    }
                    flags |= FC2_PAIR_READ_N;
                    if (n_count == 1 && n_first < 256) {
                        flags |= FC2_PAIR_READ_N1;
                        npos = (uint8_t)n_first;
                    }
                }
                if (f) {
                    const fc2_chrom_rec &c = f->chroms[pr.chrom];
                    const int64_t W = l + 2;
                    const int64_t wsA = (int64_t)pr.a_pos + e, wsB = (int64_t)pr.b_aend - e - W;
                    if (c.regular != 1) bytepath = true;
                    else if (wsA > c.size || wsA + W < 0 || wsB > c.size || wsB + W < 0) bytepath = true;
                    else {
                        auto clampg = [&](int64_t s) { return (uint64_t)std::min<int64_t>(std::max<int64_t>(s, 0), c.size) + c.gstart; };
                        if (touches_exotic(f, clampg(wsA), clampg(wsA + W)) || touches_exotic(f, clampg(wsB), clampg(wsB + W)))
                            bytepath = true;
                    }
                }
            } while (false);
            if (bytepath) {
                flags = (uint8_t)((flags & ~(FC2_PAIR_READ_N | FC2_PAIR_READ_N1)) | FC2_PAIR_BYTEPATH);
                npos = 0;
                for (auto &w : row) w = 0;
                for (auto &w : nrow) w = 0;
                ++local_bp;
            }
            pr.flags = flags;
            pr.npos = npos;
            for (uint32_t j = 0; j < rw; ++j) read_words[(uint64_t)j * stride + i] = j < 2 * kW + 1 ? row[j] : 0;
            for (uint32_t j = 0; j < nw; ++j) read_nwords[(uint64_t)j * stride + i] = j < kW ? nrow[j] : 0;
        }
        nbp += local_bp;
    });
    if (bad_chrom.load() >= 0)
        return fail(FC2_E_KEY, "pair " + std::to_string(bad_chrom.load()) +
                                   ": chromosome not in the genome index (reference KeyError, find_circ.py:193)");
    if (bad_len.load() >= 0)
        return fail(FC2_E_RANGE, "pair " + std::to_string(bad_len.load()) + ": read_part longer than " +
                                     std::to_string(FC2_MAX_READ_LEN) + " bases (fc2_result.best_x is 16-bit)");
    if (bad_rows.load() >= 0) return fail(FC2_E_PARAM, "pair " + std::to_string(bad_rows.load()) + ": read rows too narrow");
    if (bad_dist.load() >= 0) return fail(FC2_E_RANGE, "maxdist > 255 with reads whose l > 255 is not supported");
    if (n_bytepath) *n_bytepath = nbp.load();
    return FC2_OK;
}

extern "C" int fc2_window_geometry(const fc2_params *p, int max_read_len, uint32_t *pw, uint32_t *ww,
                                   uint32_t *wnw) {
    int rc = validate_params(p);
    if (rc) return rc;
    if (!pw || !ww || !wnw) return fail(FC2_E_PARAM, "fc2_window_geometry: null argument");
    const int l = std::max(0, max_read_len - 2 * eff_anchor(p));
    if (l + 2 > 128) return fail(FC2_E_RANGE, "fc2_window_geometry: window rows carry l + 2 <= 128 only");
    *pw = (uint32_t)((l + 2 + 31) / 32);
    *ww = 2 * *pw;
    *wnw = *pw;
    return FC2_OK;
}

extern "C" int fc2_pack_windows(const fc2_params *p, const fc2_fasta *f, uint64_t n, fc2_pair *pairs,
                                uint64_t *win_words, uint64_t *win_nwords, uint32_t pw, uint64_t stride,
                                int n_threads) {
    int rc = validate_params(p);
    if (rc) return rc;
    if (n && (!f || !pairs || !win_words || !win_nwords)) return fail(FC2_E_PARAM, "fc2_pack_windows: null argument");
    if (pw < 1 || pw > 4) return fail(FC2_E_RANGE, "fc2_pack_windows: pw is 1..4");
    if (stride < n) return fail(FC2_E_PARAM, "fc2_pack_windows: stride < n");
    const int e = eff_anchor(p);
    const int nch = (int)f->chroms.size();
    std::atomic<int> err{0};
    parallel_for(n, n_workers(n_threads), [&](uint64_t b, uint64_t en) {
        std::string A, B;
        for (uint64_t i = b; i < en; ++i) {
            fc2_pair &pr = pairs[i];
            uint32_t w32[16] = {0}, n32[8] = {0};
            bool anyN = false;
            const int l = (int)pr.read_len - 2 * e;
            const int W = l + 2;
            if (!(pr.flags & (FC2_PAIR_SKIP | FC2_PAIR_BYTEPATH)) && l >= 0 && W <= 32 * (int)pw &&
                (int)pr.chrom < nch) {
                const int r1 = get_upper_impl(f, (int)pr.chrom, (int64_t)pr.a_pos + e, (int64_t)pr.a_pos + e + W, A,
                                              (size_t)W + 1);
                const int r2 = get_upper_impl(f, (int)pr.chrom, (int64_t)pr.b_aend - e - W, (int64_t)pr.b_aend - e, B,
                                              (size_t)W + 1);
                if (r1 || r2) { err = r1 ? r1 : r2; continue; }
                const std::string *win[2] = {&A, &B};
                for (int x = 0; x < 2; ++x) {
                    const std::string &S = *win[x];
                    const int m = std::min<int>(W, (int)S.size());
                    for (int j = 0; j < m; ++j) {
                        const uint32_t pc = pack_code((uint8_t)S[j]);
                        const int k = j >> 5, bit = j & 31;
                        if (pc & 12u) {
                            n32[x * pw + k] |= 1u << bit;
                            anyN = true;
                            continue;
                        }
                        if (pc & 1u) w32[(2 * x) * pw + k] |= 1u << bit;
                        if (pc & 2u) w32[(2 * x + 1) * pw + k] |= 1u << bit;
                    }
                }
            }
            for (uint32_t j = 0; j < 2 * pw; ++j)
                win_words[(uint64_t)j * stride + i] = (uint64_t)w32[2 * j] | ((uint64_t)w32[2 * j + 1] << 32);
            for (uint32_t j = 0; j < pw; ++j)
                win_nwords[(uint64_t)j * stride + i] = (uint64_t)n32[2 * j] | ((uint64_t)n32[2 * j + 1] << 32);
            pr.flags = (uint8_t)((pr.flags & ~FC2_PAIR_WIN_N) | (anyN ? FC2_PAIR_WIN_N : 0u));
        }
    });
    if (err.load()) return err.load();
    return FC2_OK;
}

static inline uint64_t block_bytes(int64_t l) {
    const uint64_t lc = (uint64_t)std::max<int64_t>(0, l);
    return (16 + lc + (lc + 3) + (2 * lc + 3) + 3) & ~3ull;
}

static int fill_block(const fc2_fasta *f, int e, int64_t L, uint32_t chrom, int64_t a_pos, int64_t b_aend,
                      const uint8_t *read, uint8_t *blk, std::string &A, std::string &B) {
    const int64_t l = L - 2 * (int64_t)e;
    int64_t i0 = e, i1 = L - e;
    if (e <= 0) { i0 = std::max<int64_t>(L + e, 0); i1 = e == 0 ? 0 : std::min<int64_t>(-e, L); }
    const int32_t lenI = l < 0 ? 0 : (int32_t)std::max<int64_t>(0, i1 - i0);
    int64_t fullA = 0, fullB = 0, tailB = 0;
    A.clear(); B.clear();
    if (l >= 0) {
        const int64_t flank = l + 2;
        const int c1 = lenI == 1 ? (int)upc(read[i0]) : -1;
        int rc = get_upper_impl(f, (int)chrom, a_pos + e, a_pos + e + flank, A, (size_t)flank + 1, &fullA);
        if (rc) return rc;
        rc = get_upper_impl(f, (int)chrom, b_aend - e - flank, b_aend - e, B, (size_t)(2 * flank - 1), &fullB, c1,
                            lenI == 1 ? &tailB : nullptr);
        if (rc) return rc;
    }
    const int32_t lenA = (int32_t)std::min<int64_t>(fullA, INT32_MAX);
    const int32_t lenB = (int32_t)std::min<int64_t>(fullB, INT32_MAX);
    const int32_t tail = (int32_t)std::min<int64_t>(tailB, INT32_MAX);
    memcpy(blk, &lenI, 4);
    memcpy(blk + 4, &lenA, 4);
    memcpy(blk + 8, &lenB, 4);
    memcpy(blk + 12, &tail, 4);
    uint8_t *q = blk + 16;
    for (int64_t j = 0; j < lenI; ++j) q[j] = upc(read[i0 + j]);
    q += lenI;
    const uint64_t lc = (uint64_t)std::max<int64_t>(0, l);
    memcpy(q, A.data(), std::min<size_t>(A.size(), lc + 3));
    q += lc + 3;
    memcpy(q, B.data(), std::min<size_t>(B.size(), 2 * lc + 3));
    return FC2_OK;
}

extern "C" int fc2_bytepath_size(const fc2_params *p, uint64_t n, const fc2_pair *pairs, uint64_t *m, uint64_t *arena_bytes) {
    int rc = validate_params(p);
    if (rc) return rc;
    const int e = eff_anchor(p);
    uint64_t mm = 0, bytes = 0;
    for (uint64_t i = 0; i < n; ++i) {
        if (!(pairs[i].flags & FC2_PAIR_BYTEPATH)) continue;
        bytes += block_bytes((int64_t)pairs[i].read_len - 2 * e);
        ++mm;
    }
    if (m) *m = mm;
    if (arena_bytes) *arena_bytes = bytes;
    return FC2_OK;
}

extern "C" int fc2_bytepath_fill(const fc2_params *p, const fc2_fasta *f, uint64_t n, const uint8_t *reads,
                                 const uint64_t *read_off, const fc2_pair *pairs, uint64_t *index, fc2_pair *bpairs,
                                 uint64_t *off, uint8_t *arena) {
    int rc = validate_params(p);
    if (rc) return rc;
    const int e = eff_anchor(p);
    uint64_t k = 0, pos = 0;
    std::string A, B;
    for (uint64_t i = 0; i < n; ++i) {
        const fc2_pair &pr = pairs[i];
        if (!(pr.flags & FC2_PAIR_BYTEPATH)) continue;
        if ((rc = fill_block(f, e, pr.read_len, pr.chrom, pr.a_pos, pr.b_aend, reads + read_off[i], arena + pos, A, B)))
            return rc;
        index[k] = i;
        bpairs[k] = pr;
        off[k] = pos;
        pos += block_bytes((int64_t)pr.read_len - 2 * e);
        ++k;
    }
    return FC2_OK;
}

extern "C" int fc2_long_geometry(const fc2_params *p, uint64_t n, const fc2_long_pair *pairs, uint64_t *arena_bytes,
                                 uint64_t *tie_off) {
    int rc = validate_params(p);
    if (rc) return rc;
    if (n && !pairs) return fail(FC2_E_PARAM, "fc2_long_geometry: null pairs");
    const int e = eff_anchor(p);
    uint64_t bytes = 0, words = 0;
    for (uint64_t i = 0; i < n; ++i) {
        const int64_t l = (int64_t)pairs[i].read_len - 2 * e;
        bytes += block_bytes(l);
        if (tie_off) tie_off[i] = words;
        words += 2 * (uint64_t)((std::max<int64_t>(l, 0) + 2 + 63) / 64);
    }
    if (tie_off) tie_off[n] = words;
    if (arena_bytes) *arena_bytes = bytes;
    return FC2_OK;
}

extern "C" int fc2_long_fill(const fc2_params *p, const fc2_fasta *f, uint64_t n, const uint8_t *reads,
                             const fc2_long_pair *pairs, uint64_t *off, uint8_t *arena) {
    int rc = validate_params(p);
    if (rc) return rc;
    if (n && (!reads || !pairs || !off || !arena)) return fail(FC2_E_PARAM, "fc2_long_fill: null argument");
    const int e = eff_anchor(p);
    const int nch = f ? (int)f->chroms.size() : 0;
    uint64_t pos = 0;
    std::string A, B;
    for (uint64_t i = 0; i < n; ++i) {
        const fc2_long_pair &pr = pairs[i];
        if (pr.read_len > (uint32_t)INT32_MAX) return fail(FC2_E_RANGE, "fc2_long_fill: read part of 2^31 bases or more");
        off[i] = pos;
        const int64_t l = (int64_t)pr.read_len - 2 * e;
        if (!(pr.flags & FC2_PAIR_SKIP)) {
            if (f && (int)pr.chrom >= nch)
                return fail(FC2_E_KEY, "long pair " + std::to_string(i) +
                                           ": chromosome not in the genome index (reference KeyError, find_circ.py:193)");
            if ((rc = fill_block(f, e, pr.read_len, pr.chrom, pr.a_pos, pr.b_aend, reads + pr.read_off, arena + pos, A, B)))
                return rc;
        } else {
            memset(arena + pos, 0, 16);
        }
        pos += block_bytes(l);
    }
    return FC2_OK;
}

extern "C" int fc2_result_expand(const fc2_params *p, const void *words, int width, uint64_t n,
                                 const fc2_result_escape *esc, uint64_t n_esc, fc2_result *out, int n_threads) {
    if (int rc = fc2::validate_params(p)) return rc;
    if (p->noncanonical) return fc2::fail(FC2_E_PARAM, "fc2_result_expand: the compact forms hold canonical-mode results only");
    if (width != 2 && width != 4) return fc2::fail(FC2_E_PARAM, "fc2_result_expand: width is 2 or 4");
    if ((n && (!words || !out)) || (n_esc && !esc)) return fc2::fail(FC2_E_PARAM, "fc2_result_expand: bad args");
    std::atomic<uint64_t> flagged{0};
    auto escaped = [&](uint64_t i) {
        return width == 2 ? (((const uint16_t *)words)[i] & 0x7Fu) == FC2_R16_ESCAPE
                          : (((const uint32_t *)words)[i] & FC2_R32_ESCAPE) != 0;
    };
    parallel_for(n, n_workers(n_threads), [&](uint64_t b, uint64_t e) {
        uint64_t f = 0;
        uint64_t *o = (uint64_t *)out;
        if (width == 2) {
            const uint16_t *w = (const uint16_t *)words;
            for (uint64_t i = b; i < e; ++i) {
                const uint16_t c = w[i];
                const bool x = (c & 0x7Fu) == FC2_R16_ESCAPE;
                f += x;
                o[i] = x ? 0 : fc2::r16_unpack(c);
            }
        } else {
            const uint32_t *w = (const uint32_t *)words;
            for (uint64_t i = b; i < e; ++i) {
                const uint32_t c = w[i];
                f += c >> 31;
                o[i] = (c & FC2_R32_ESCAPE) ? 0 : fc2::r32_unpack(c);
            }
        }
        flagged += f;
    });
    if (flagged.load() != n_esc)
        return fc2::fail(FC2_E_FORMAT, "fc2_result_expand: " + std::to_string(flagged.load()) + " escaped words, " +
                                           std::to_string(n_esc) + " escapes");
    std::vector<uint64_t> idx(n_esc);
    for (uint64_t k = 0; k < n_esc; ++k) {
        if (esc[k].index >= n || !escaped(esc[k].index))
            return fc2::fail(FC2_E_FORMAT, "fc2_result_expand: escape " + std::to_string(k) + " has no escaped word");
        idx[k] = esc[k].index;
        out[esc[k].index] = esc[k].result;
    }
    std::sort(idx.begin(), idx.end());
    if (std::adjacent_find(idx.begin(), idx.end()) != idx.end())
        return fc2::fail(FC2_E_FORMAT, "fc2_result_expand: an escaped word has two escapes");
    return FC2_OK;
}
```

include/fc2_bp.h:

```cpp
#ifndef FC2_BP_H
#define FC2_BP_H

#include <stddef.h>
#include <stdint.h>

#ifdef __cplusplus
extern "C" {
#endif

#define FC2_ABI_VERSION 1

#define FC2_OK        0
#define FC2_E_PARAM  -1
#define FC2_E_HIP    -2
#define FC2_E_FORMAT -3
#define FC2_E_RANGE  -4
#define FC2_E_IO     -5
#define FC2_E_KEY    -6
#define FC2_E_OS     -7

typedef struct fc2_params {
    int32_t asize;
    int32_t margin;
    int32_t maxdist;
    uint8_t noncanonical;
    uint8_t strandpref;
    uint8_t allhits;
    uint8_t _pad;
} fc2_params;

#define FC2_PAIR_BACKSPLICE  0x01u
#define FC2_PAIR_PRIMARY_REV 0x02u
#define FC2_PAIR_READ_N      0x04u
#define FC2_PAIR_BYTEPATH    0x08u
#define FC2_PAIR_SKIP        0x10u
#define FC2_PAIR_WIN_N       0x20u
#define FC2_PAIR_READ_N1     0x40u

typedef struct fc2_pair {
    int32_t  a_pos;
    int32_t  b_aend;
    uint32_t chrom;
    uint16_t read_len;
    uint8_t  flags;
    uint8_t  npos;
} fc2_pair;

#define FC2_MAX_READ_LEN 32767

#define FC2_RES_MINUS       0x0001u
#define FC2_RES_GTAG_SHIFT  1
#define FC2_RES_GTAG_MASK   0x1FFEu
#define FC2_RES_ERR_KEY     0x2000u
#define FC2_RES_ERR_WIN     0x4000u
#define FC2_RES_DONE        0x8000u

typedef struct fc2_result {
    int16_t  best_x;
    uint8_t  dist;
    uint8_t  ov;
    uint16_t n_ties;
    uint16_t info;
} fc2_result;

#define FC2_R32_ESCAPE 0x80000000u
#define FC2_R16_ESCAPE 0x007Fu
typedef struct fc2_result_escape {
    uint64_t   index;
    fc2_result result;
} fc2_result_escape;
int fc2_result_compact_launch(const fc2_params *p, const fc2_result *results, uint64_t n, int width, void *words,
                              fc2_result_escape *esc, uint32_t esc_cap, uint32_t *esc_count, void *stream);
int fc2_host_device_pointer(void *host, void **dev);
int fc2_result_expand(const fc2_params *p, const void *words, int width, uint64_t n, const fc2_result_escape *esc,
                      uint64_t n_esc, fc2_result *out, int n_threads);

typedef struct fc2_genome_view {
    const uint64_t *units;
    const uint64_t *nplane;
    const uint32_t *ncoarse;
    const uint64_t *chrom_start;
    const int64_t  *chrom_size;
    uint64_t n_units;
    uint32_t n_chrom;
    uint32_t dummy;
    const uint64_t *units_twin;
    const uint32_t *nsuper;
    uint32_t nsuper_shift;
    uint32_t nsuper_words;
    const uint32_t *wt;
    uint64_t wt_bytes;
    uint64_t wt_twin_off;
} fc2_genome_view;

typedef struct fc2_batch_view {
    const fc2_pair *pairs;
    const uint64_t *read_words;
    const uint64_t *read_nwords;
    uint64_t n;
    uint64_t stride;
    uint32_t rw;
    uint32_t nw;
    int32_t  max_l;
    uint32_t layout;
    const uint64_t *win_words;
    const uint64_t *win_nwords;
    uint32_t ww;
    uint32_t wnw;
} fc2_batch_view;
#define FC2_BATCH_LOCUS_ORDERED 0x1u
#define FC2_BATCH_FORM_STAGED  0x02u
#define FC2_BATCH_FORM_PLAIN   0x04u
#define FC2_BATCH_FORM_UNITS   0x08u
#define FC2_BATCH_FORM_TWOLANE 0x10u
#define FC2_BATCH_FORM_TRI     0x20u
#define FC2_BATCH_FORM_FIVE    0x40u
#define FC2_BATCH_FORM_WAVE    0x80u

typedef struct fc2_bytes_view {
    const uint64_t *index;
    const fc2_pair *pairs;
    const uint8_t  *arena;
    const uint64_t *off;
    uint64_t m;
} fc2_bytes_view;

typedef struct fc2_long_pair {
    uint64_t read_off;
    uint32_t read_len;
    uint32_t chrom;
    int32_t  a_pos;
    int32_t  b_aend;
    uint8_t  flags;
    uint8_t  _pad[7];
} fc2_long_pair;

typedef struct fc2_long_result {
    int32_t  best_x;
    uint32_t n_ties;
    uint8_t  dist, ov;
    uint16_t info;
    uint32_t _pad;
} fc2_long_result;

int         fc2_abi_version(void);
const char *fc2_last_error(void);
int         fc2_device_count(int *count);
int         fc2_host_register(void *ptr, uint64_t bytes);
int         fc2_host_unregister(void *ptr);

int         fc2_gather_windows_launch(const fc2_params *p, const fc2_genome_view *g, const fc2_batch_view *b,
                                      fc2_pair *pairs, uint64_t *win_words, uint64_t *win_nwords, uint32_t pw,
                                      void *stream);

int         fc2_probe_pattern_launch(const fc2_params *p, const fc2_genome_view *g, const fc2_batch_view *b,
                                     uint64_t *out, void *stream);

#define FC2_TUNE_STREAM_NT 1
#define FC2_TUNE_KERNEL32  2
#define FC2_TUNE_XCD_SWIZZLE 3
#define FC2_TUNE_REORDER_ROUNDS 4
#define FC2_TUNE_REORDER_NT 5
#define FC2_TUNE_TWIN 6
#define FC2_TUNE_STAGE 7
#define FC2_TUNE_EXTRA_LDS 9
#define FC2_TUNE_PERSIST 10
#define FC2_TUNE_WORDS 11
#define FC2_TUNE_STAGE_BLOCK 13
#define FC2_TUNE_TRI 14
#define FC2_TUNE_REORDER_SHIFT 12
int         fc2_set_tuning(int key, int value);
int         fc2_get_tuning(int key, int *value);

int         fc2_max_fast_l(void);
int         fc2_batch_geometry(const fc2_params *p, int32_t max_read_len,
                               uint32_t *rw, uint32_t *nw, uint32_t *tw);

int fc2_bp_scan_launch(const fc2_params *p, const fc2_genome_view *g, const fc2_batch_view *b,
                       fc2_result *results, uint64_t *tiemask, uint32_t tw, void *stream);

typedef struct fc2_compact_out {
    int32_t  width;
    uint32_t esc_cap;
    void    *words;
    fc2_result_escape *esc;
    uint32_t *esc_count;
    uint32_t *count_out;
} fc2_compact_out;
int fc2_bp_scan_compact_launch(const fc2_params *p, const fc2_genome_view *g, const fc2_batch_view *b,
                               const fc2_compact_out *co, void *stream);
int fc2_bp_scan_bytes_launch(const fc2_params *p, const fc2_bytes_view *v, fc2_result *results,
                             uint64_t *tiemask, uint32_t tw, uint64_t stride, void *stream);

typedef struct fc2_reorder_info {
    uint64_t n;
    uint64_t workspace_bytes;
    uint32_t shift;
    uint32_t n_buckets;
    uint32_t bucket_bits;
    uint32_t n_chunks;
    uint32_t n_groups;
    uint32_t chunk;
} fc2_reorder_info;
int fc2_reorder_plan(const fc2_genome_view *g, uint64_t n, fc2_reorder_info *info);
int fc2_reorder_launch(const fc2_reorder_info *info, const fc2_genome_view *g, const fc2_batch_view *in,
                       fc2_pair *pairs_out, uint64_t *read_words_out, uint64_t *read_nwords_out,
                       uint32_t *slot_out, void *workspace, void *stream);
typedef struct fc2_fasta fc2_fasta;

int  fc2_fasta_open(const char *path, int write_index, fc2_fasta **out);
void fc2_fasta_close(fc2_fasta *f);
int  fc2_fasta_n_chrom(const fc2_fasta *f);
int  fc2_fasta_chrom(const fc2_fasta *f, int i, const char **name, int64_t *size,
                     int64_t *ofs, int64_t *ldata, int64_t *skip, int *regular);
int  fc2_fasta_find(const fc2_fasta *f, const char *name);
int  fc2_fasta_get_upper(const fc2_fasta *f, int chrom, int64_t start, int64_t end,
                         uint8_t *out, int64_t cap, int64_t *len);
int  fc2_fasta_layout(const fc2_fasta *f, uint64_t *n_units, uint64_t *n_coarse_words,
                      uint64_t *chrom_start );
int  fc2_fasta_pack(const fc2_fasta *f, uint64_t *units, uint64_t *nplane, uint32_t *ncoarse,
                    uint64_t *n_exotic, int n_threads);
int  fc2_fasta_prepack(fc2_fasta *f, int n_threads);

int fc2_pack_pairs(const fc2_params *p, const fc2_fasta *f, uint64_t n,
                   const uint8_t *reads, const uint64_t *read_off,
                   fc2_pair *pairs_io, uint64_t *read_words, uint32_t rw,
                   uint64_t *read_nwords, uint32_t nw, uint64_t stride,
                   uint64_t *n_bytepath, int n_threads);

int fc2_window_geometry(const fc2_params *p, int max_read_len, uint32_t *pw, uint32_t *ww, uint32_t *wnw);
int fc2_pack_windows(const fc2_params *p, const fc2_fasta *f, uint64_t n, fc2_pair *pairs_io,
                     uint64_t *win_words, uint64_t *win_nwords, uint32_t pw, uint64_t stride, int n_threads);

int fc2_bytepath_size(const fc2_params *p, uint64_t n, const fc2_pair *pairs, uint64_t *m,
                      uint64_t *arena_bytes);
int fc2_bytepath_fill(const fc2_params *p, const fc2_fasta *f, uint64_t n,
                      const uint8_t *reads, const uint64_t *read_off, const fc2_pair *pairs,
                      uint64_t *index, fc2_pair *bpairs, uint64_t *off, uint8_t *arena);

int fc2_long_geometry(const fc2_params *p, uint64_t n, const fc2_long_pair *pairs, uint64_t *arena_bytes,
                      uint64_t *tie_off);
int fc2_long_fill(const fc2_params *p, const fc2_fasta *f, uint64_t n, const uint8_t *reads, const fc2_long_pair *pairs,
                  uint64_t *off, uint8_t *arena);
int fc2_bp_scan_long_launch(const fc2_params *p, uint64_t n, const fc2_long_pair *pairs, const uint64_t *off,
                            const uint8_t *arena, const uint64_t *tie_off, fc2_long_result *results, uint64_t *ties,
                            void *stream);

typedef struct fc2_synth_cfg {
    uint64_t seed;
    int32_t  len_min, len_max;
    float    p_planted;
    float    p_minus_site;
    float    p_backsplice;
    float    mut_rate;
    float    n_rate;
    float    p_clip;
    int32_t  span_min, span_max;
    int32_t  locus_ordered;
    float    p_three_seg;
    uint64_t first;
} fc2_synth_cfg;

int fc2_synth_genome_launch(uint64_t seed, uint64_t *units, uint64_t *nplane, uint32_t *ncoarse,
                            uint64_t n_units, const int64_t *n_lo, const int64_t *n_hi,
                            uint32_t n_intervals, void *stream);
int fc2_wtab_geometry(uint64_t n_units, uint64_t *bytes, uint64_t *twin_off);
int fc2_wtab_launch(const uint64_t *units, uint64_t n_units, uint32_t *wt, void *stream);
int fc2_twin_launch(const uint64_t *units, uint64_t n_units, uint64_t *units_twin, void *stream);
int fc2_nsuper_geometry(uint64_t n_units, uint32_t *shift, uint32_t *words);
int fc2_nsuper_launch(const uint32_t *ncoarse, uint64_t n_units, uint32_t *nsuper, void *stream);
int fc2_coarse_launch(const uint64_t *nplane, uint32_t *ncoarse, uint64_t n_units, void *stream);

int fc2_synth_pairs_launch(const fc2_params *p, const fc2_synth_cfg *cfg, const fc2_genome_view *g,
                           const int64_t *chrom_cum, uint64_t n, fc2_pair *pairs,
                           uint64_t *read_words, uint32_t rw, uint64_t *read_nwords, uint32_t nw,
                           uint64_t stride, int32_t *truth, void *stream);

#ifdef __cplusplus
}
#endif
#endif
```

include/fc2_ctx.h:

```cpp
#ifndef FC2_CTX_H
#define FC2_CTX_H

#include "fc2_bp.h"

#ifdef __cplusplus
extern "C" {
#endif

typedef struct fc2_ctx fc2_ctx;

int  fc2_ctx_create(int device, fc2_ctx **out);
int  fc2_ctx_create_sibling(const fc2_ctx *src, fc2_ctx **out);
void fc2_ctx_destroy(fc2_ctx *ctx);

int  fc2_ctx_genome_load(fc2_ctx *ctx, const fc2_fasta *fa, int n_threads);
int  fc2_ctx_genome_view(const fc2_ctx *ctx, fc2_genome_view *out);

int  fc2_ctx_scan_async(fc2_ctx *ctx, const fc2_params *p, uint64_t n, const uint8_t *reads,
                        const uint64_t *read_off, const fc2_pair *pairs, fc2_result *results,
                        uint64_t *tiemask, uint32_t tw, int n_threads);
int  fc2_ctx_sync(fc2_ctx *ctx);

int  fc2_ctx_scan_long(fc2_ctx *ctx, const fc2_params *p, uint64_t n, const uint8_t *reads, const fc2_long_pair *pairs,
                       fc2_long_result *results, uint64_t *ties);

void *fc2_ctx_stream(const fc2_ctx *ctx);
const char *fc2_ctx_last_error(const fc2_ctx *ctx);

#ifdef __cplusplus
}
#endif

#endif
```

Before: 24.10 billion.

## Move read-row bit packing from host to a GPU kernel in ctx scan

The host no longer packs reads into 2-bit row words and N-masks. It now stages the raw read bytes into a compact buffer, copies those to the device, and runs a new row_pack kernel that builds the rows there. The host-side memset, the packing work and the larger H2D transfer of packed rows are replaced by a smaller raw-byte copy plus a GPU pass. Reads with exotic characters are counted with an atomic, and if any exist the whole batch is packed again on the host, which adds a fallback path and a sync.

```diff
diff --git a/find_circ2_amd/_native.py b/find_circ2_amd/_native.py
--- a/find_circ2_amd/_native.py
+++ b/find_circ2_amd/_native.py
@@ -134,7 +134,7 @@
     "fc2_result_compact_launch", "fc2_result_expand", "fc2_bp_scan_compact_launch", "fc2_host_device_pointer",
     "fc2_fasta_open", "fc2_fasta_close", "fc2_fasta_n_chrom", "fc2_fasta_chrom", "fc2_fasta_find",
     "fc2_fasta_get_upper", "fc2_fasta_layout", "fc2_fasta_pack", "fc2_fasta_prepack",
-    "fc2_pack_pairs", "fc2_bytepath_size", "fc2_bytepath_fill", "fc2_window_geometry", "fc2_pack_windows",
+    "fc2_pack_pairs", "fc2_stage_size", "fc2_stage_pairs", "fc2_row_pack_launch", "fc2_bytepath_size", "fc2_bytepath_fill", "fc2_window_geometry", "fc2_pack_windows",
     "fc2_gather_windows_launch", "fc2_long_geometry", "fc2_long_fill", "fc2_bp_scan_long_launch",
     "fc2_synth_genome_launch", "fc2_coarse_launch", "fc2_twin_launch", "fc2_wtab_geometry", "fc2_wtab_launch",
     "fc2_nsuper_geometry", "fc2_nsuper_launch", "fc2_synth_pairs_launch",
@@ -150,7 +150,7 @@
     "fc2_caller_set_reads_gz", "fc2_caller_close_reads", "fc2_caller_set_reads_gz_device", "fc2_caller_reads_gz_counts",
     "fc2_deflate_launch", "fc2_deflate_scratch_bytes", "fc2_gpu_gzip", "fc2_gpu_gzip_bound", "fc2_caller_set_reads_gz_device_tuning",
     "fc2_ctx_create", "fc2_ctx_create_sibling", "fc2_ctx_destroy", "fc2_ctx_genome_load", "fc2_ctx_genome_view", "fc2_ctx_scan_async",
-    "fc2_ctx_sync", "fc2_ctx_scan_long", "fc2_ctx_stream", "fc2_ctx_last_error",
+    "fc2_ctx_sync", "fc2_ctx_pack_counts", "fc2_ctx_scan_long", "fc2_ctx_stream", "fc2_ctx_last_error",
 ]
 
 
@@ -199,7 +199,7 @@
     srcdir = os.path.join(_HERE, "csrc")
     srcs = [os.path.join(srcdir, f) for f in ("fc2_kernels.hip", "fc2_scan32.hip", "fc2_reorder.hip", "fc2_inflate.hip",
                                               "fc2_deflate.hip", "fc2_deflate_gpu.hip", "fc2_deflate_gpu.h", "fc2_devcrc.h",
-                                              "fc2_gzpieces.h", "fc2_scan32.h",
+                                              "fc2_gzpieces.h", "fc2_scan32.h", "fc2_rowpack.hip", "fc2_packcode.h",
                                               "fc2_host.cpp", "fc2_ingest.cpp", "fc2_ingest_impl.h", "fc2_caller.cpp",
                                               "fc2_bamout.cpp", "fc2_bamout.h", "fc2_ctx.cpp", "fc2_hostmem.h",
                                               "fc2_common.h", "Makefile")]
@@ -250,6 +250,10 @@
         "fc2_fasta_prepack": (ctypes.c_int, [vp, ctypes.c_int]),
         "fc2_pack_pairs": (ctypes.c_int, [P(Params), vp, u64, vp, vp, vp, vp, u32, vp, u32, u64, P(u64),
                                           ctypes.c_int]),
+        "fc2_stage_size": (ctypes.c_int, [u64, vp, vp, P(u64), P(i32)]),
+        "fc2_stage_pairs": (ctypes.c_int, [P(Params), vp, u64, vp, vp, vp, u32, u32, vp, vp, P(u64), P(i32),
+                                           ctypes.c_int]),
+        "fc2_row_pack_launch": (ctypes.c_int, [P(Params), u64, vp, vp, vp, vp, u32, vp, u32, u64, vp, vp]),
         "fc2_bytepath_size": (ctypes.c_int, [P(Params), u64, vp, P(u64), P(u64)]),
         "fc2_window_geometry": (ctypes.c_int, [P(Params), ctypes.c_int, P(u32), P(u32), P(u32)]),
         "fc2_pack_windows": (ctypes.c_int, [P(Params), vp, u64, vp, vp, vp, u32, u64, ctypes.c_int]),
@@ -324,6 +328,7 @@
         "fc2_ctx_genome_view": (ctypes.c_int, [vp, P(GenomeView)]),
         "fc2_ctx_scan_async": (ctypes.c_int, [vp, P(Params), u64, vp, vp, vp, vp, vp, u32, ctypes.c_int]),
         "fc2_ctx_sync": (ctypes.c_int, [vp]),
+        "fc2_ctx_pack_counts": (ctypes.c_int, [vp, P(u64), P(u64)]),
         "fc2_ctx_scan_long": (ctypes.c_int, [vp, P(Params), u64, vp, vp, vp, vp]),
         "fc2_ctx_stream": (vp, [vp]),
         "fc2_ctx_last_error": (ctypes.c_char_p, [vp]),
diff --git a/find_circ2_amd/csrc/fc2_ctx.cpp b/find_circ2_amd/csrc/fc2_ctx.cpp
--- a/find_circ2_amd/csrc/fc2_ctx.cpp
+++ b/find_circ2_amd/csrc/fc2_ctx.cpp
@@ -77,14 +77,24 @@
     fc2_genome_view gv{};
     DevBuf units, nplane, ncoarse, cstart, csize, twin, nsuper, wt;
     fc2::MappedWords h_units, h_nplane;
-    HostBuf h_pairs, h_words, h_nwords, h_res, h_tm, h_bidx, h_bpairs, h_boff, h_arena;
-    DevBuf d_pairs, d_words, d_nwords, d_res, d_tm, d_bidx, d_bpairs, d_boff, d_arena;
+    HostBuf h_pairs, h_reads, h_soff, h_cnt, h_words, h_nwords, h_res, h_tm, h_bidx, h_bpairs, h_boff, h_arena;
+    DevBuf d_pairs, d_reads, d_soff, d_cnt, d_words, d_nwords, d_res, d_tm, d_bidx, d_bpairs, d_boff, d_arena;
     bool pending = false;
     uint64_t n = 0;
-    uint32_t tw = 0;
+    uint32_t tw = 0, rw = 0, nw = 0;
     bool allhits = false;
+    fc2_params params{};
+    int n_threads = 0;
     fc2_result *out_res = nullptr;
     uint64_t *out_tm = nullptr;
+    uint64_t last_exotic = 0, n_redone = 0;
+
+    std::vector<HostBuf *> host_bufs() {
+        return {&h_pairs, &h_reads, &h_soff, &h_cnt, &h_words, &h_nwords, &h_res, &h_tm, &h_bidx, &h_bpairs, &h_boff, &h_arena};
+    }
+    std::vector<DevBuf *> dev_bufs() {
+        return {&d_pairs, &d_reads, &d_soff, &d_cnt, &d_words, &d_nwords, &d_res, &d_tm, &d_bidx, &d_bpairs, &d_boff, &d_arena};
+    }
 
     void free_genome() {
         if (!borrowed)
@@ -117,6 +127,80 @@
     if (!bytes) return FC2_OK;
     const hipError_t e = hipMemcpyAsync(d.p, src, bytes, hipMemcpyHostToDevice, s);
     return e == hipSuccess ? FC2_OK : hip_fail(e, "hipMemcpyAsync H2D");
+}
+
+int queue_scan(fc2_ctx *c, const uint8_t *reads, const uint64_t *read_off, uint64_t n_bytepath, int max_l) {
+    const fc2_params *p = &c->params;
+    const uint64_t n = c->n;
+    const uint32_t tw = c->tw;
+    const hipStream_t s = c->stream;
+    const fc2_pair *hp = c->h_pairs.as<fc2_pair>();
+    const size_t tmw = c->allhits ? (size_t)tw * n : 0;
+    int rc;
+    if (tmw && hipMemsetAsync(c->d_tm.p, 0, tmw * 8, s) != hipSuccess) return fc2::fail(FC2_E_HIP, "tie-mask memset");
+    fc2_batch_view bv{};
+    bv.pairs = c->d_pairs.as<const fc2_pair>();
+    bv.read_words = c->d_words.as<const uint64_t>();
+    bv.read_nwords = c->d_nwords.as<const uint64_t>();
+    bv.n = n;
+    bv.stride = n;
+    bv.rw = c->rw;
+    bv.nw = c->nw;
+    bv.max_l = max_l;
+    bv.layout = 0;
+    uint64_t *dtm = tmw ? c->d_tm.as<uint64_t>() : nullptr;
+    if ((rc = fc2_bp_scan_launch(p, &c->gv, &bv, c->d_res.as<fc2_result>(), dtm, tw, s))) return rc;
+    if (n_bytepath) {
+        uint64_t m = 0, arena = 0;
+        if ((rc = fc2_bytepath_size(p, n, hp, &m, &arena))) return rc;
+        if ((rc = c->h_bidx.reserve(m * 8, "byte-path index")) || (rc = c->h_bpairs.reserve(m * sizeof(fc2_pair), "byte-path pairs")) ||
+            (rc = c->h_boff.reserve(m * 8, "byte-path offsets")) || (rc = c->h_arena.reserve(std::max<uint64_t>(arena, 16), "byte-path arena")) ||
+            (rc = c->d_bidx.reserve(m * 8, "byte-path index")) || (rc = c->d_bpairs.reserve(m * sizeof(fc2_pair), "byte-path pairs")) ||
+            (rc = c->d_boff.reserve(m * 8, "byte-path offsets")) || (rc = c->d_arena.reserve(std::max<uint64_t>(arena, 16), "byte-path arena")))
+            return rc;
+        if ((rc = fc2_bytepath_fill(p, c->fa, n, reads, read_off, hp, c->h_bidx.as<uint64_t>(), c->h_bpairs.as<fc2_pair>(),
+                                    c->h_boff.as<uint64_t>(), c->h_arena.as<uint8_t>())))
+            return rc;
+        if ((rc = h2d(c->d_bidx, c->h_bidx.p, m * 8, s)) || (rc = h2d(c->d_bpairs, c->h_bpairs.p, m * sizeof(fc2_pair), s)) ||
+            (rc = h2d(c->d_boff, c->h_boff.p, m * 8, s)) || (rc = h2d(c->d_arena, c->h_arena.p, arena, s)))
+            return rc;
+        fc2_bytes_view v{c->d_bidx.as<const uint64_t>(), c->d_bpairs.as<const fc2_pair>(), c->d_arena.as<const uint8_t>(),
+                         c->d_boff.as<const uint64_t>(), m};
+        if ((rc = fc2_bp_scan_bytes_launch(p, &v, c->d_res.as<fc2_result>(), dtm, tw, n, s))) return rc;
+    }
+    hipError_t he = hipMemcpyAsync(c->h_res.p, c->d_res.p, n * 8, hipMemcpyDeviceToHost, s);
+    if (he == hipSuccess && tmw) he = hipMemcpyAsync(c->h_tm.p, c->d_tm.p, tmw * 8, hipMemcpyDeviceToHost, s);
+    if (he != hipSuccess) return hip_fail(he, "hipMemcpyAsync D2H");
+    return FC2_OK;
+}
+
+int redo_on_host(fc2_ctx *c) {
+    const uint64_t n = c->n;
+    const uint32_t rw = c->rw, nw = c->nw;
+    int rc;
+    if ((rc = c->h_words.reserve((size_t)rw * n * 8, "read-row staging")) || (rc = c->h_nwords.reserve((size_t)nw * n * 8, "N-row staging")))
+        return rc;
+    memset(c->h_words.p, 0, (size_t)rw * n * 8);
+    memset(c->h_nwords.p, 0, (size_t)nw * n * 8);
+    fc2_pair *hp = c->h_pairs.as<fc2_pair>();
+    const uint8_t *reads = c->h_reads.as<const uint8_t>();
+    const uint64_t *off = c->h_soff.as<const uint64_t>();
+    uint64_t n_bytepath = 0;
+    if ((rc = fc2_pack_pairs(&c->params, c->fa, n, reads, off, hp, c->h_words.as<uint64_t>(), rw, c->h_nwords.as<uint64_t>(), nw, n,
+                             &n_bytepath, c->n_threads)))
+        return rc;
+    const int e = fc2::eff_anchor(&c->params);
+    int max_l = 0;
+    for (uint64_t i = 0; i < n; ++i)
+        if (!(hp[i].flags & (FC2_PAIR_BYTEPATH | FC2_PAIR_SKIP))) max_l = std::max(max_l, (int)hp[i].read_len - 2 * e);
+    const hipStream_t s = c->stream;
+    if (!(rc = h2d(c->d_pairs, hp, n * sizeof(fc2_pair), s)) && !(rc = h2d(c->d_words, c->h_words.p, (size_t)rw * n * 8, s)) &&
+        !(rc = h2d(c->d_nwords, c->h_nwords.p, (size_t)nw * n * 8, s)))
+        rc = queue_scan(c, reads, off, n_bytepath, max_l);
+    const std::string msg = rc ? fc2_last_error() : "";
+    const hipError_t he = hipStreamSynchronize(s);
+    if (rc) return fc2::fail(rc, msg);
+    return he == hipSuccess ? FC2_OK : hip_fail(he, "fc2_ctx_sync (host pack)");
 }
 
 }
@@ -164,12 +248,8 @@
     if (!c) return;
     if (hipSetDevice(c->device) == hipSuccess && c->stream) (void)hipStreamSynchronize(c->stream);
     c->free_genome();
-    for (HostBuf *b : {&c->h_pairs, &c->h_words, &c->h_nwords, &c->h_res, &c->h_tm, &c->h_bidx, &c->h_bpairs,
-                       &c->h_boff, &c->h_arena})
-        b->release();
-    for (DevBuf *b : {&c->d_pairs, &c->d_words, &c->d_nwords, &c->d_res, &c->d_tm, &c->d_bidx, &c->d_bpairs,
-                      &c->d_boff, &c->d_arena})
-        b->release();
+    for (HostBuf *b : c->host_bufs()) b->release();
+    for (DevBuf *b : c->dev_bufs()) b->release();
     if (c->stream) (void)hipStreamDestroy(c->stream);
     delete c;
 }
@@ -292,75 +372,53 @@
         c->pending = true;
         return FC2_OK;
     }
-    int max_len = 0;
-    for (uint64_t i = 0; i < n; ++i) max_len = std::max<int>(max_len, pairs[i].read_len);
+    c->params = *p;
+    c->n_threads = n_threads;
+    if ((rc = c->h_soff.reserve(n * 8, "read-offset staging"))) return keep(c, rc);
+    uint64_t *soff = c->h_soff.as<uint64_t>();
+    uint64_t rbytes = 0;
+    int32_t max_len = 0;
+    if ((rc = fc2_stage_size(n, pairs, soff, &rbytes, &max_len))) return keep(c, rc);
     uint32_t rw = 0, nw = 0, tw_need = 0;
     if ((rc = fc2_batch_geometry(p, max_len, &rw, &nw, &tw_need))) return keep(c, rc);
     if (c->allhits && tw < tw_need)
         return keep(c, fc2::fail(FC2_E_PARAM, "fc2_ctx_scan_async: tie mask of " + std::to_string(tw) + " words per pair, " +
                                                   std::to_string(tw_need) + " needed"));
+    c->rw = rw;
+    c->nw = nw;
     const size_t tmw = c->allhits ? (size_t)tw * n : 0;
-    if ((rc = c->h_pairs.reserve(n * sizeof(fc2_pair), "pair staging")) || (rc = c->h_words.reserve((size_t)rw * n * 8, "read-row staging")) ||
-        (rc = c->h_nwords.reserve((size_t)nw * n * 8, "N-row staging")) || (rc = c->h_res.reserve(n * 8, "result staging")) ||
+    if ((rc = c->h_pairs.reserve(n * sizeof(fc2_pair), "pair staging")) || (rc = c->h_reads.reserve(rbytes + 16, "read staging")) ||
+        (rc = c->h_cnt.reserve(8, "exotic-read count")) || (rc = c->h_res.reserve(n * 8, "result staging")) ||
         (tmw && (rc = c->h_tm.reserve(tmw * 8, "tie-mask staging"))) || (rc = c->d_pairs.reserve(n * sizeof(fc2_pair), "pairs")) ||
-        (rc = c->d_words.reserve((size_t)rw * n * 8, "read rows")) || (rc = c->d_nwords.reserve((size_t)nw * n * 8, "N rows")) ||
-        (rc = c->d_res.reserve(n * 8, "results")) || (tmw && (rc = c->d_tm.reserve(tmw * 8, "tie mask"))))
+        (rc = c->d_reads.reserve(rbytes + 16, "reads")) || (rc = c->d_soff.reserve(n * 8, "read offsets")) ||
+        (rc = c->d_cnt.reserve(8, "exotic-read count")) || (rc = c->d_words.reserve((size_t)rw * n * 8, "read rows")) ||
+        (rc = c->d_nwords.reserve((size_t)nw * n * 8, "N rows")) || (rc = c->d_res.reserve(n * 8, "results")) ||
+        (tmw && (rc = c->d_tm.reserve(tmw * 8, "tie mask"))))
         return keep(c, rc);
     memcpy(c->h_pairs.p, pairs, n * sizeof(fc2_pair));
-    memset(c->h_words.p, 0, (size_t)rw * n * 8);
-    memset(c->h_nwords.p, 0, (size_t)nw * n * 8);
     fc2_pair *hp = c->h_pairs.as<fc2_pair>();
     uint64_t n_bytepath = 0;
-    if ((rc = fc2_pack_pairs(p, c->fa, n, reads, read_off, hp, c->h_words.as<uint64_t>(), rw, c->h_nwords.as<uint64_t>(), nw,
-                             n, &n_bytepath, n_threads)))
+    int32_t max_l = 0;
+    if ((rc = fc2_stage_pairs(p, c->fa, n, reads, read_off, hp, rw, nw, soff, c->h_reads.as<uint8_t>(), &n_bytepath, &max_l,
+                              n_threads)))
         return keep(c, rc);
-    const int e = fc2::eff_anchor(p);
-    int max_l = 0;
-    for (uint64_t i = 0; i < n; ++i)
-        if (!(hp[i].flags & (FC2_PAIR_BYTEPATH | FC2_PAIR_SKIP))) max_l = std::max(max_l, (int)hp[i].read_len - 2 * e);
+    *c->h_cnt.as<uint64_t>() = 0;
     const hipStream_t s = c->stream;
     auto abandon = [&](int code) {
         const std::string msg = fc2_last_error();
         (void)hipStreamSynchronize(s);
         return keep(c, fc2::fail(code, msg));
     };
-    if ((rc = h2d(c->d_pairs, hp, n * sizeof(fc2_pair), s)) || (rc = h2d(c->d_words, c->h_words.p, (size_t)rw * n * 8, s)) ||
-        (rc = h2d(c->d_nwords, c->h_nwords.p, (size_t)nw * n * 8, s)))
+    if ((rc = h2d(c->d_pairs, hp, n * sizeof(fc2_pair), s)) || (rc = h2d(c->d_soff, soff, n * 8, s)) ||
+        (rc = h2d(c->d_reads, c->h_reads.p, rbytes, s)))
         return abandon(rc);
-    if (tmw && hipMemsetAsync(c->d_tm.p, 0, tmw * 8, s) != hipSuccess) return abandon(fc2::fail(FC2_E_HIP, "tie-mask memset"));
-    fc2_batch_view bv{};
-    bv.pairs = c->d_pairs.as<const fc2_pair>();
-    bv.read_words = c->d_words.as<const uint64_t>();
-    bv.read_nwords = c->d_nwords.as<const uint64_t>();
-    bv.n = n;
-    bv.stride = n;
-    bv.rw = rw;
-    bv.nw = nw;
-    bv.max_l = max_l;
-    bv.layout = 0;
-    uint64_t *dtm = tmw ? c->d_tm.as<uint64_t>() : nullptr;
-    if ((rc = fc2_bp_scan_launch(p, &c->gv, &bv, c->d_res.as<fc2_result>(), dtm, tw, s))) return abandon(rc);
-    if (n_bytepath) {
-        uint64_t m = 0, arena = 0;
-        if ((rc = fc2_bytepath_size(p, n, hp, &m, &arena))) return abandon(rc);
-        if ((rc = c->h_bidx.reserve(m * 8, "byte-path index")) || (rc = c->h_bpairs.reserve(m * sizeof(fc2_pair), "byte-path pairs")) ||
-            (rc = c->h_boff.reserve(m * 8, "byte-path offsets")) || (rc = c->h_arena.reserve(std::max<uint64_t>(arena, 16), "byte-path arena")) ||
-            (rc = c->d_bidx.reserve(m * 8, "byte-path index")) || (rc = c->d_bpairs.reserve(m * sizeof(fc2_pair), "byte-path pairs")) ||
-            (rc = c->d_boff.reserve(m * 8, "byte-path offsets")) || (rc = c->d_arena.reserve(std::max<uint64_t>(arena, 16), "byte-path arena")))
-            return abandon(rc);
-        if ((rc = fc2_bytepath_fill(p, c->fa, n, reads, read_off, hp, c->h_bidx.as<uint64_t>(), c->h_bpairs.as<fc2_pair>(),
-                                    c->h_boff.as<uint64_t>(), c->h_arena.as<uint8_t>())))
-            return abandon(rc);
-        if ((rc = h2d(c->d_bidx, c->h_bidx.p, m * 8, s)) || (rc = h2d(c->d_bpairs, c->h_bpairs.p, m * sizeof(fc2_pair), s)) ||
-            (rc = h2d(c->d_boff, c->h_boff.p, m * 8, s)) || (rc = h2d(c->d_arena, c->h_arena.p, arena, s)))
-            return abandon(rc);
-        fc2_bytes_view v{c->d_bidx.as<const uint64_t>(), c->d_bpairs.as<const fc2_pair>(), c->d_arena.as<const uint8_t>(),
-                         c->d_boff.as<const uint64_t>(), m};
-        if ((rc = fc2_bp_scan_bytes_launch(p, &v, c->d_res.as<fc2_result>(), dtm, tw, n, s))) return abandon(rc);
-    }
-    hipError_t he = hipMemcpyAsync(c->h_res.p, c->d_res.p, n * 8, hipMemcpyDeviceToHost, s);
-    if (he == hipSuccess && tmw) he = hipMemcpyAsync(c->h_tm.p, c->d_tm.p, tmw * 8, hipMemcpyDeviceToHost, s);
-    if (he != hipSuccess) return abandon(hip_fail(he, "hipMemcpyAsync D2H"));
+    if (hipMemsetAsync(c->d_cnt.p, 0, 8, s) != hipSuccess) return abandon(fc2::fail(FC2_E_HIP, "exotic-read count memset"));
+    if ((rc = fc2_row_pack_launch(p, n, c->d_reads.as<const uint8_t>(), c->d_soff.as<const uint64_t>(), c->d_pairs.as<fc2_pair>(),
+                                  c->d_words.as<uint64_t>(), rw, c->d_nwords.as<uint64_t>(), nw, n, c->d_cnt.as<uint32_t>(), s)))
+        return abandon(rc);
+    if ((rc = queue_scan(c, reads, read_off, n_bytepath, max_l))) return abandon(rc);
+    if (hipMemcpyAsync(c->h_cnt.p, c->d_cnt.p, 4, hipMemcpyDeviceToHost, s) != hipSuccess)
+        return abandon(fc2::fail(FC2_E_HIP, "exotic-read count D2H"));
     c->pending = true;
     return FC2_OK;
 }
@@ -375,9 +433,21 @@
     const hipError_t e = hipStreamSynchronize(c->stream);
     if (e != hipSuccess) return keep(c, hip_fail(e, "fc2_ctx_sync"));
     if (c->n) {
+        c->last_exotic = *c->h_cnt.as<uint32_t>();
+        if (c->last_exotic) {
+            ++c->n_redone;
+            if ((rc = redo_on_host(c))) return keep(c, rc);
+        }
         memcpy(c->out_res, c->h_res.p, c->n * 8);
         if (c->allhits) memcpy(c->out_tm, c->h_tm.p, (size_t)c->tw * c->n * 8);
     }
+    return FC2_OK;
+}
+
+extern "C" int fc2_ctx_pack_counts(const fc2_ctx *c, uint64_t *last_exotic, uint64_t *n_redone) {
+    if (!c) return fc2::fail(FC2_E_PARAM, "fc2_ctx_pack_counts: null context");
+    if (last_exotic) *last_exotic = c->last_exotic;
+    if (n_redone) *n_redone = c->n_redone;
     return FC2_OK;
 }
 
diff --git a/find_circ2_amd/csrc/fc2_host.cpp b/find_circ2_amd/csrc/fc2_host.cpp
--- a/find_circ2_amd/csrc/fc2_host.cpp
+++ b/find_circ2_amd/csrc/fc2_host.cpp
@@ -21,6 +21,7 @@
 #include "fc2_common.h"
 #include "fc2_compact.h"
 #include "fc2_hostmem.h"
+#include "fc2_packcode.h"
 
 namespace fc2 {
 
@@ -69,24 +70,10 @@
 
 static inline uint8_t upc(uint8_t c) { return (c >= 'a' && c <= 'z') ? (uint8_t)(c - 32) : c; }
 
-static inline int bclass(uint8_t c) {
-    switch (upc(c)) {
-        case 'A': return 0;
-        case 'C': return 1;
-        case 'G': return 2;
-        case 'T': return 3;
-        case 'N': return 4;
-        default: return 5;
-    }
-}
-
 struct PackTable {
     uint8_t t[256];
     PackTable() {
-        for (int c = 0; c < 256; ++c) {
-            const int cl = bclass((uint8_t)c);
-            t[c] = (uint8_t)(cl < 4 ? cl : cl == 4 ? 4 : 4 | 8);
-        }
+        for (int c = 0; c < 256; ++c) t[c] = (uint8_t)pack_code_of((uint8_t)c);
     }
 };
 static const PackTable kPackTable;
@@ -131,13 +118,6 @@
 #else
 static const bool kHaveAvx2 = (__builtin_cpu_init(), __builtin_cpu_supports("avx2"));
 #endif
-
-static inline bool acgt8(uint64_t u) {
-    auto zero = [](uint64_t y) { return ~(((y & 0x7F7F7F7F7F7F7F7Full) + 0x7F7F7F7F7F7F7F7Full) | y | 0x7F7F7F7F7F7F7F7Full); };
-    const uint64_t m = zero(u ^ 0x4141414141414141ull) | zero(u ^ 0x4343434343434343ull) |
-                       zero(u ^ 0x4747474747474747ull) | zero(u ^ 0x5454545454545454ull);
-    return m == 0x8080808080808080ull;
-}
 
 static inline bool py_isspace(uint8_t c) {
     return c == ' ' || c == '\t' || c == '\n' || c == '\r' || c == '\v' || c == '\f';
@@ -725,6 +705,16 @@
     if (f->exotic.empty() || g1 <= g0) return false;
     auto it = std::lower_bound(f->exotic.begin(), f->exotic.end(), g0);
     return it != f->exotic.end() && *it < g1;
+}
+
+static bool windows_need_bytes(const fc2_fasta *f, const fc2_pair &pr, int e, int l) {
+    const fc2_chrom_rec &c = f->chroms[pr.chrom];
+    const int64_t W = l + 2;
+    const int64_t wsA = (int64_t)pr.a_pos + e, wsB = (int64_t)pr.b_aend - e - W;
+    if (c.regular != 1) return true;
+    if (wsA > c.size || wsA + W < 0 || wsB > c.size || wsB + W < 0) return true;
+    auto clampg = [&](int64_t s) { return (uint64_t)std::min<int64_t>(std::max<int64_t>(s, 0), c.size) + c.gstart; };
+    return touches_exotic(f, clampg(wsA), clampg(wsA + W)) || touches_exotic(f, clampg(wsB), clampg(wsB + W));
 }
 
 extern "C" int fc2_pack_pairs(const fc2_params *p, const fc2_fasta *f, uint64_t n, const uint8_t *reads,
@@ -812,18 +802,7 @@
                         npos = (uint8_t)n_first;
                     }
                 }
-                if (f) {
-                    const fc2_chrom_rec &c = f->chroms[pr.chrom];
-                    const int64_t W = l + 2;
-                    const int64_t wsA = (int64_t)pr.a_pos + e, wsB = (int64_t)pr.b_aend - e - W;
-                    if (c.regular != 1) bytepath = true;
-                    else if (wsA > c.size || wsA + W < 0 || wsB > c.size || wsB + W < 0) bytepath = true;
-                    else {
-                        auto clampg = [&](int64_t s) { return (uint64_t)std::min<int64_t>(std::max<int64_t>(s, 0), c.size) + c.gstart; };
-                        if (touches_exotic(f, clampg(wsA), clampg(wsA + W)) || touches_exotic(f, clampg(wsB), clampg(wsB + W)))
-                            bytepath = true;
-                    }
-                }
+                if (f && windows_need_bytes(f, pr, e, l)) bytepath = true;
             } while (false);
             if (bytepath) {
                 flags = (uint8_t)((flags & ~(FC2_PAIR_READ_N | FC2_PAIR_READ_N1)) | FC2_PAIR_BYTEPATH);
@@ -848,6 +827,85 @@
     if (bad_rows.load() >= 0) return fail(FC2_E_PARAM, "pair " + std::to_string(bad_rows.load()) + ": read rows too narrow");
     if (bad_dist.load() >= 0) return fail(FC2_E_RANGE, "maxdist > 255 with reads whose l > 255 is not supported");
     if (n_bytepath) *n_bytepath = nbp.load();
+    return FC2_OK;
+}
+
+extern "C" int fc2_stage_size(uint64_t n, const fc2_pair *pairs, uint64_t *stage_off, uint64_t *stage_bytes,
+                              int32_t *max_read_len) {
+    if (n && (!pairs || !stage_off)) return fail(FC2_E_PARAM, "fc2_stage_size: null argument");
+    uint64_t pos = 0;
+    int max_len = 0;
+    for (uint64_t i = 0; i < n; ++i) {
+        stage_off[i] = pos;
+        max_len = std::max<int>(max_len, pairs[i].read_len);
+        if (!(pairs[i].flags & FC2_PAIR_SKIP)) pos += pairs[i].read_len;
+    }
+    if (stage_bytes) *stage_bytes = pos;
+    if (max_read_len) *max_read_len = max_len;
+    return FC2_OK;
+}
+
+extern "C" int fc2_stage_pairs(const fc2_params *p, const fc2_fasta *f, uint64_t n, const uint8_t *reads,
+                               const uint64_t *read_off, fc2_pair *pairs, uint32_t rw, uint32_t nw,
+                               const uint64_t *stage_off, uint8_t *stage, uint64_t *n_bytepath, int32_t *max_l,
+                               int n_threads) {
+    int rc = validate_params(p);
+    if (rc) return rc;
+    if (n && (!reads || !read_off || !pairs || !stage_off || !stage)) return fail(FC2_E_PARAM, "fc2_stage_pairs: null argument");
+    if (f && !f->packed) return fail(FC2_E_PARAM, "fc2_stage_pairs: genome must be packed first (fc2_fasta_pack)");
+    const int e = eff_anchor(p);
+    const int T = (int)std::min<uint64_t>((uint64_t)n_workers(n_threads), std::max<uint64_t>(1, n >> 15));
+    std::atomic<uint64_t> nbp{0};
+    std::atomic<int> ml{0};
+    std::atomic<int64_t> bad_chrom{-1}, bad_rows{-1}, bad_dist{-1}, bad_len{-1};
+    const int nch = f ? (int)f->chroms.size() : 0;
+    const int maxdist = p->maxdist;
+    parallel_for(n, T, [&](uint64_t b, uint64_t en) {
+        uint64_t local_bp = 0;
+        int local_ml = 0;
+        for (uint64_t i = b; i < en; ++i) {
+            fc2_pair &pr = pairs[i];
+            uint8_t flags = (uint8_t)(pr.flags & (FC2_PAIR_BACKSPLICE | FC2_PAIR_PRIMARY_REV | FC2_PAIR_SKIP));
+            const int L = pr.read_len;
+            const int l = L - 2 * e;
+            bool bytepath = false, scanned = false;
+            do {
+                if (flags & FC2_PAIR_SKIP) break;
+                if (L > FC2_MAX_READ_LEN) { int64_t x = -1; bad_len.compare_exchange_strong(x, (int64_t)i); break; }
+                if (f && (int)pr.chrom >= nch) { int64_t x = -1; bad_chrom.compare_exchange_strong(x, (int64_t)i); break; }
+                if (l < 0) break;
+                if (maxdist > 255 && l > 255) { int64_t x = -1; bad_dist.compare_exchange_strong(x, (int64_t)i); }
+                if (e <= 0) { bytepath = true; break; }
+                if (l > kMaxFastL) { bytepath = true; break; }
+                if ((uint64_t)2 * l > (uint64_t)rw * 64 || (uint64_t)l > (uint64_t)nw * 64) {
+                    int64_t x = -1; bad_rows.compare_exchange_strong(x, (int64_t)i); break;
+                }
+                if (f && windows_need_bytes(f, pr, e, l)) bytepath = true;
+                scanned = !bytepath;
+            } while (false);
+            if (bytepath) {
+                flags |= FC2_PAIR_BYTEPATH;
+                ++local_bp;
+            }
+            if (scanned) local_ml = std::max(local_ml, l);
+            pr.flags = flags;
+            pr.npos = 0;
+            if (!(flags & FC2_PAIR_SKIP)) memcpy(stage + stage_off[i], reads + read_off[i], (size_t)L);
+        }
+        nbp += local_bp;
+        int cur = ml.load();
+        while (local_ml > cur && !ml.compare_exchange_weak(cur, local_ml)) {}
+    });
+    if (bad_chrom.load() >= 0)
+        return fail(FC2_E_KEY, "pair " + std::to_string(bad_chrom.load()) +
+                                   ": chromosome not in the genome index (reference KeyError, find_circ.py:193)");
+    if (bad_len.load() >= 0)
+        return fail(FC2_E_RANGE, "pair " + std::to_string(bad_len.load()) + ": read_part longer than " +
+                                     std::to_string(FC2_MAX_READ_LEN) + " bases (fc2_result.best_x is 16-bit)");
+    if (bad_rows.load() >= 0) return fail(FC2_E_PARAM, "pair " + std::to_string(bad_rows.load()) + ": read rows too narrow");
+    if (bad_dist.load() >= 0) return fail(FC2_E_RANGE, "maxdist > 255 with reads whose l > 255 is not supported");
+    if (n_bytepath) *n_bytepath = nbp.load();
+    if (max_l) *max_l = ml.load();
     return FC2_OK;
 }
 
diff --git a/find_circ2_amd/csrc/fc2_packcode.h b/find_circ2_amd/csrc/fc2_packcode.h
--- /dev/null
+++ b/find_circ2_amd/csrc/fc2_packcode.h
@@ -0,0 +1,28 @@
+#pragma once
+#include <hip/hip_runtime.h>
+#include <stdint.h>
+
+namespace fc2 {
+
+__host__ __device__ inline uint32_t pack_code_of(uint8_t c) {
+    const uint8_t u = (c >= 'a' && c <= 'z') ? (uint8_t)(c - 32) : c;
+    return u == 'A' ? 0u : u == 'C' ? 1u : u == 'G' ? 2u : u == 'T' ? 3u : u == 'N' ? 4u : 12u;
+}
+
+__host__ __device__ inline uint64_t zero_bytes(uint64_t y) {
+    return ~(((y & 0x7F7F7F7F7F7F7F7Full) + 0x7F7F7F7F7F7F7F7Full) | y | 0x7F7F7F7F7F7F7F7Full);
+}
+
+__host__ __device__ inline bool acgt8(uint64_t u) {
+    const uint64_t m = zero_bytes(u ^ 0x4141414141414141ull) | zero_bytes(u ^ 0x4343434343434343ull) |
+                       zero_bytes(u ^ 0x4747474747474747ull) | zero_bytes(u ^ 0x5454545454545454ull);
+    return m == 0x8080808080808080ull;
+}
+
+__host__ __device__ inline void acgt8_bits(uint64_t x, uint64_t &lo8, uint64_t &hi8) {
+    const uint64_t v = ((x >> 2) ^ (x >> 1)) & 0x0303030303030303ull;
+    lo8 = ((v & 0x0101010101010101ull) * 0x0102040810204080ull) >> 56;
+    hi8 = (((v >> 1) & 0x0101010101010101ull) * 0x0102040810204080ull) >> 56;
+}
+
+}
diff --git a/find_circ2_amd/csrc/fc2_rowpack.hip b/find_circ2_amd/csrc/fc2_rowpack.hip
--- /dev/null
+++ b/find_circ2_amd/csrc/fc2_rowpack.hip
@@ -0,0 +1,132 @@
+#include <hip/hip_runtime.h>
+#include <stdint.h>
+
+#include <string>
+
+#include "../../include/fc2_bp.h"
+#include "fc2_common.h"
+#include "fc2_packcode.h"
+
+namespace {
+
+constexpr int kBlock = 256;
+
+struct RowWord {
+    uint64_t lo, hi, n;
+    uint32_t any;
+};
+
+__device__ inline RowWord row_word(const uint8_t *src, int l, int k) {
+    RowWord r{0, 0, 0, 0};
+    const unsigned a = (unsigned)((uintptr_t)src & 7u);
+    const uint64_t *w = reinterpret_cast<const uint64_t *>(src - a) + 8 * k;
+    const int left = l - 64 * k;
+#pragma unroll 1
+    for (int g = 0; g < 8 && 8 * g < left; ++g) {
+        const int v = left - 8 * g < 8 ? left - 8 * g : 8;
+        uint64_t x = w[g] >> (8 * a);
+        if (a + (unsigned)v > 8u) x |= w[g + 1] << (64 - 8 * a);
+        uint64_t lo8 = 0, hi8 = 0, n8 = 0;
+        if (v == 8 && fc2::acgt8(x & 0xDFDFDFDFDFDFDFDFull)) {
+            fc2::acgt8_bits(x, lo8, hi8);
+        } else {
+            for (int b = 0; b < v; ++b) {
+                const uint32_t pc = fc2::pack_code_of((uint8_t)(x >> (8 * b)));
+                if (pc & 4u) n8 |= 1ull << b;
+                else {
+                    lo8 |= (uint64_t)(pc & 1u) << b;
+                    hi8 |= (uint64_t)((pc >> 1) & 1u) << b;
+                }
+                r.any |= pc;
+            }
+        }
+        r.lo |= lo8 << (8 * g);
+        r.hi |= hi8 << (8 * g);
+        r.n |= n8 << (8 * g);
+    }
+    return r;
+}
+
+__global__ __launch_bounds__(kBlock) void row_pack_kernel(int e, uint64_t n, const uint8_t *__restrict__ reads,
+                                                          const uint64_t *__restrict__ read_off, fc2_pair *__restrict__ pairs,
+                                                          uint64_t *__restrict__ rows, uint32_t rw,
+                                                          uint64_t *__restrict__ nrows, uint32_t nw, uint64_t stride,
+                                                          uint32_t *__restrict__ n_exotic) {
+    const uint64_t i = (uint64_t)blockIdx.x * kBlock + threadIdx.x;
+    if (i >= n) return;
+    fc2_pair pr = pairs[i];
+    uint8_t flags = (uint8_t)(pr.flags & (FC2_PAIR_BACKSPLICE | FC2_PAIR_PRIMARY_REV | FC2_PAIR_SKIP | FC2_PAIR_BYTEPATH));
+    uint8_t npos = 0;
+    const int l = (int)pr.read_len - 2 * e;
+    uint32_t jr = 0, jn = 0;
+    bool pack = !(flags & (FC2_PAIR_SKIP | FC2_PAIR_BYTEPATH)) && l >= 0;
+    if (pack && (e <= 0 || l > fc2::kMaxFastL)) {
+        flags |= FC2_PAIR_BYTEPATH;
+        pack = false;
+    }
+    if (pack && ((uint64_t)2 * l > (uint64_t)rw * 64 || (uint64_t)l > (uint64_t)nw * 64)) pack = false;
+    if (pack) {
+        const uint8_t *src = reads + read_off[i] + e;
+        const int nlw = (l + 63) / 64, sh = l & 63, wo = l >> 6;
+        uint32_t any = 0;
+        int n_count = 0, n_first = 0;
+        uint64_t carry = 0;
+        for (int k = 0; k < nlw; ++k) {
+            const RowWord r = row_word(src, l, k);
+            any |= r.any;
+            if (r.n) {
+                if (n_count == 0) n_first = k * 64 + __builtin_ctzll(r.n);
+                n_count += __builtin_popcountll(r.n);
+            }
+            if (k == wo) carry = r.lo;
+        }
+        if (any & 8u) {
+            atomicAdd(n_exotic, 1u);
+            flags |= FC2_PAIR_BYTEPATH;
+        } else {
+            if (any & 4u) {
+                flags |= FC2_PAIR_READ_N;
+                if (n_count == 1 && n_first < 256) {
+                    flags |= FC2_PAIR_READ_N1;
+                    npos = (uint8_t)n_first;
+                }
+            }
+            for (int k = 0; k < nlw; ++k) {
+                const RowWord r = row_word(src, l, k);
+                if (k < wo) rows[(uint64_t)k * stride + i] = r.lo;
+                nrows[(uint64_t)k * stride + i] = r.n;
+                rows[(uint64_t)(wo + k) * stride + i] = carry | (sh ? r.hi << sh : r.hi);
+                carry = sh ? r.hi >> (64 - sh) : 0;
+            }
+            jr = (uint32_t)(wo + nlw);
+            jn = (uint32_t)nlw;
+            if (sh && jr < rw) rows[(uint64_t)jr++ * stride + i] = carry;
+        }
+    }
+    for (; jr < rw; ++jr) rows[(uint64_t)jr * stride + i] = 0;
+    for (; jn < nw; ++jn) nrows[(uint64_t)jn * stride + i] = 0;
+    pr.flags = flags;
+    pr.npos = npos;
+    pairs[i] = pr;
+}
+
+}
+
+extern "C" int fc2_row_pack_launch(const fc2_params *p, uint64_t n, const uint8_t *reads, const uint64_t *read_off,
+                                   fc2_pair *pairs, uint64_t *read_words, uint32_t rw, uint64_t *read_nwords,
+                                   uint32_t nw, uint64_t stride, uint32_t *n_exotic, void *stream) {
+    int rc = fc2::validate_params(p);
+    if (rc) return rc;
+    if (n == 0) return FC2_OK;
+    if (!reads || !read_off || !pairs || !read_words || !read_nwords || !n_exotic)
+        return fc2::fail(FC2_E_PARAM, "fc2_row_pack_launch: null argument");
+    if (stride < n) return fc2::fail(FC2_E_PARAM, "fc2_row_pack_launch: stride < n");
+    if (rw == 0 || nw == 0) return fc2::fail(FC2_E_PARAM, "fc2_row_pack_launch: rw and nw are at least 1");
+    if ((uintptr_t)reads & 7u) return fc2::fail(FC2_E_PARAM, "fc2_row_pack_launch: reads must be 8-byte aligned");
+    if (n > (uint64_t)0x7FFFFFFF * kBlock) return fc2::fail(FC2_E_RANGE, "fc2_row_pack_launch: too many pairs");
+    hipLaunchKernelGGL(row_pack_kernel, dim3((unsigned)((n + kBlock - 1) / kBlock)), dim3(kBlock), 0, (hipStream_t)stream,
+                       fc2::eff_anchor(p), n, reads, read_off, pairs, read_words, rw, read_nwords, nw, stride, n_exotic);
+    const hipError_t e = hipGetLastError();
+    if (e != hipSuccess) return fc2::fail(FC2_E_HIP, std::string("row_pack_kernel launch: ") + hipGetErrorString(e));
+    return FC2_OK;
+}
diff --git a/include/fc2_bp.h b/include/fc2_bp.h
--- a/include/fc2_bp.h
+++ b/include/fc2_bp.h
@@ -228,6 +228,16 @@
                    uint64_t *read_nwords, uint32_t nw, uint64_t stride,
                    uint64_t *n_bytepath, int n_threads);
 
+int fc2_stage_size(uint64_t n, const fc2_pair *pairs, uint64_t *stage_off, uint64_t *stage_bytes,
+                   int32_t *max_read_len);
+int fc2_stage_pairs(const fc2_params *p, const fc2_fasta *f, uint64_t n, const uint8_t *reads,
+                    const uint64_t *read_off, fc2_pair *pairs_io, uint32_t rw, uint32_t nw,
+                    const uint64_t *stage_off, uint8_t *stage, uint64_t *n_bytepath, int32_t *max_l,
+                    int n_threads);
+int fc2_row_pack_launch(const fc2_params *p, uint64_t n, const uint8_t *reads, const uint64_t *read_off,
+                        fc2_pair *pairs_io, uint64_t *read_words, uint32_t rw, uint64_t *read_nwords,
+                        uint32_t nw, uint64_t stride, uint32_t *n_exotic, void *stream);
+
 int fc2_window_geometry(const fc2_params *p, int max_read_len, uint32_t *pw, uint32_t *ww, uint32_t *wnw);
 int fc2_pack_windows(const fc2_params *p, const fc2_fasta *f, uint64_t n, fc2_pair *pairs_io,
                      uint64_t *win_words, uint64_t *win_nwords, uint32_t pw, uint64_t stride, int n_threads);
diff --git a/include/fc2_ctx.h b/include/fc2_ctx.h
--- a/include/fc2_ctx.h
+++ b/include/fc2_ctx.h
@@ -20,6 +20,7 @@
                         const uint64_t *read_off, const fc2_pair *pairs, fc2_result *results,
                         uint64_t *tiemask, uint32_t tw, int n_threads);
 int  fc2_ctx_sync(fc2_ctx *ctx);
+int  fc2_ctx_pack_counts(const fc2_ctx *ctx, uint64_t *last_exotic, uint64_t *n_redone);
 
 int  fc2_ctx_scan_long(fc2_ctx *ctx, const fc2_params *p, uint64_t n, const uint8_t *reads, const fc2_long_pair *pairs,
                        fc2_long_result *results, uint64_t *ties);
```

Result: no change. 23.92 billion (-0.7%).
